# UZ-SLAMLab/DefSLAM

Measured on AMD Instinct MI355X. Metric: SfT GN iters/sec (500-node mesh, 1k matches), higher is better.
Workload: dtype f64

## Files before the change

defslam_amd/csrc/dsh_api.cpp:

```cpp
#include <hip/hip_runtime.h>

#include <algorithm>
#include <cmath>
#include <cstdio>
#include <cstdlib>
#include <cstring>

#include <memory>
#include <mutex>
#include <string>
#include <vector>

#include "dsh_sft_ctx.h"

#include "mapping_launch.h"

#ifdef DSH_LAB
#include "../../include/defslam_hip_debug.h"
#endif

LdsMarks g_lds_marks[64];
std::mutex g_lds_mu;

using dsh::Tcw_from_pose7;

dsh_ctx_base* dsh_base(dsh_ctx* ctx) { return static_cast<dsh_ctx_base*>(ctx); }
const dsh::TemplateHost* dsh_facet_template(dsh_ctx_base* c) {
  const dsh_ctx* x = static_cast<const dsh_ctx*>(c);
  return x && x->tmpl.valid && x->tmpl.F > 0 ? &x->tmpl : nullptr;
}

namespace {

void drop_graphs(dsh_ctx* c) {
  if (!c->host_only && c->stream) (void)hipStreamSynchronize(c->stream);
  for (auto& g : c->graphs)
    if (g->d_base) (void)hipFree(g->d_base);
  c->graphs.clear();
  c->packed.clear();
}

int upload_template(dsh_ctx* c) {
  c->B = 0;
  c->ran = false;
  drop_graphs(c);
  if (c->host_only) return DSH_OK;
  const dsh::TemplateHost& t = c->tmpl;
  Arena a;
  const size_t o_xyz0 = a.take(sizeof(double) * 3 * t.n);
  const size_t o_ptr = a.take(sizeof(int32_t) * (t.n + 1));
  const size_t o_idx = a.take(sizeof(int32_t) * t.nbr_idx.size());
  const size_t o_w = a.take(sizeof(double) * t.nbr_w.size());
  const size_t o_sw = a.take(sizeof(double) * t.n);
  const size_t o_k0 = a.take(sizeof(double) * t.n);
  if (c->d_tmpl) { (void)hipFree(c->d_tmpl); c->d_tmpl = nullptr; }
  HIPCHK(c, hipMalloc((void**)&c->d_tmpl, a.size));
  c->d_tmpl_bytes = a.size;
  std::vector<char> st(a.size, 0);
  std::memcpy(&st[o_xyz0], t.xyz0.data(), sizeof(double) * 3 * t.n);
  std::memcpy(&st[o_ptr], t.nbr_ptr.data(), sizeof(int32_t) * (t.n + 1));
  std::memcpy(&st[o_idx], t.nbr_idx.data(), sizeof(int32_t) * t.nbr_idx.size());
  std::memcpy(&st[o_w], t.nbr_w.data(), sizeof(double) * t.nbr_w.size());
  std::memcpy(&st[o_sw], t.nbr_sumw.data(), sizeof(double) * t.n);
  std::memcpy(&st[o_k0], t.k0.data(), sizeof(double) * t.n);
  HIPCHK(c, hipMemcpy(c->d_tmpl, st.data(), a.size, hipMemcpyHostToDevice));
  c->dt.xyz0 = (const double*)(c->d_tmpl + o_xyz0);
  c->dt.nbr_ptr = (const int32_t*)(c->d_tmpl + o_ptr);
  c->dt.nbr_idx = (const int32_t*)(c->d_tmpl + o_idx);
  c->dt.nbr_w = (const double*)(c->d_tmpl + o_w);
  c->dt.nbr_sumw = (const double*)(c->d_tmpl + o_sw);
  c->dt.k0 = (const double*)(c->d_tmpl + o_k0);
  return DSH_OK;
}

template <class T>
size_t reserve(Arena& a, const std::vector<T>& v) { return a.take(sizeof(T) * v.size()); }
template <class T>
void put(char* st, size_t off, const std::vector<T>& v) {
  if (!v.empty()) std::memcpy(st + off, v.data(), sizeof(T) * v.size());
}

int graph_for(dsh_ctx* c, const std::vector<uint8_t>& opt, dsh::SftGraph** out, std::string& err) {
  uint64_t h = 1469598103934665603ull;
  for (uint8_t b : opt) { h ^= b; h *= 1099511628211ull; }
  for (auto& g : c->graphs)
    if (g->opt_hash == h && g->opt == opt) { g->last_use = c->upload_serial; *out = g.get(); return DSH_OK; }
  if (c->graphs.size() >= 64) {
    if (!c->host_only && c->stream) (void)hipStreamSynchronize(c->stream);
    auto& gs = c->graphs;
    for (size_t i = 0; i < gs.size();) {
      if (gs[i]->last_use != c->upload_serial) {
        if (gs[i]->d_base) (void)hipFree(gs[i]->d_base);
        gs.erase(gs.begin() + i);
      } else {
        i++;
      }
    }
  }
  std::unique_ptr<dsh::SftGraph> g(new dsh::SftGraph());
  const int rc = dsh::build_graph(c->tmpl, opt, *g, err);
  if (rc != DSH_OK) return rc;
  g->last_use = c->upload_serial;
  if (!c->host_only) {
    Arena a;
    auto& o = g->o;
    o.act = reserve(a, g->act); o.actnode = reserve(a, g->actnode); o.star_node = reserve(a, g->star_node); o.star_sL = reserve(a, g->star_sL);
    o.str_nodes = reserve(a, g->str_nodes); o.str_L0 = reserve(a, g->str_L0); o.off_ptr = reserve(a, g->off_ptr); o.off_rc = reserve(a, g->off_rc);
    o.sh_ptr = reserve(a, g->sh_ptr); o.sh_rec = reserve(a, g->sh_rec); o.sh_cf = reserve(a, g->sh_cf); o.tmask = reserve(a, g->tmask);
    o.hgather = reserve(a, g->hgather);
    o.hgatherT = reserve(a, g->hgatherT);
    std::vector<char> st(a.size, 0);
    put(st.data(), o.act, g->act); put(st.data(), o.actnode, g->actnode); put(st.data(), o.star_node, g->star_node); put(st.data(), o.star_sL, g->star_sL);
    put(st.data(), o.str_nodes, g->str_nodes); put(st.data(), o.str_L0, g->str_L0); put(st.data(), o.off_ptr, g->off_ptr); put(st.data(), o.off_rc, g->off_rc);
    put(st.data(), o.sh_ptr, g->sh_ptr); put(st.data(), o.sh_rec, g->sh_rec); put(st.data(), o.sh_cf, g->sh_cf); put(st.data(), o.tmask, g->tmask);
    put(st.data(), o.hgather, g->hgather);
    put(st.data(), o.hgatherT, g->hgatherT);
    if (hipMalloc((void**)&g->d_base, a.size) != hipSuccess) { err = "out of device memory (graph)"; return DSH_ERR_HIP; }
    g->d_bytes = a.size;
    if (hipMemcpy(g->d_base, st.data(), a.size, hipMemcpyHostToDevice) != hipSuccess) { (void)hipFree(g->d_base); err = "graph upload failed"; return DSH_ERR_HIP; }
  }
  *out = g.get();
  c->graphs.push_back(std::move(g));
  return DSH_OK;
}

int pack_problem(dsh_ctx* c, const dsh_sft_frame& f, Packed& P, std::string& err) {
  const dsh::TemplateHost& t = c->tmpl;
  std::vector<uint8_t> viewed, opt;
  int rc = dsh::frame_active_set(t, f, viewed, opt, err);
  if (rc != DSH_OK) return rc;
  rc = graph_for(c, opt, &P.g, err);
  if (rc != DSH_OK) return rc;
  const dsh::SftGraph& g = *P.g;
  rc = dsh::pack_frame(t, g, f, viewed, P.f, err);
  if (rc != DSH_OK) return rc;
  SftDev& h = P.h;
  h = SftDev{};
  h.n = t.n; h.nA = g.nA; h.Dn = 3 * g.nA; h.kd = g.kd; h.ldh = h.kd + 1;
  h.M = f.M; h.V = P.f.V; h.S = g.S; h.Es = g.Es; h.noff = g.noff; h.max_iters = f.max_iters; h.mode = 0;
  h.fx = f.K[0]; h.fy = f.K[1]; h.cx = f.K[2]; h.cy = f.K[3];
  h.w_ref = f.reg_temp / std::pow(t.median_L, 2);
  h.w_curv = f.reg_lap / (double)g.nA;
  h.w_str = g.Es > 0 ? f.reg_inex / (double)g.Es : 0.0;
  const float deltaMono = (float)std::sqrt(5.991);
  h.hub_delta = (double)deltaMono;
  h.hub_dsqr = h.hub_delta * h.hub_delta;
  return DSH_OK;
}

int run_rounds_enqueue(dsh_ctx* c);
int run_rounds(dsh_ctx* c) {
  const int rc = run_rounds_enqueue(c);
  if (rc != DSH_OK)
    for (int s = 0; s < c->plan.n_sub; s++) if (c->sub_stream[s]) (void)hipStreamSynchronize(c->sub_stream[s]);
  return rc;
}
int run_rounds_enqueue(dsh_ctx* c) {
  const int B = c->B, S = c->plan.n_sub;
  int b0[kSftMaxSub + 1];
  for (int s = 0; s <= S; s++) b0[s] = (int)((long long)B * s / S);
  int tail_below = -1;
  if (S == 1 && c->opt.tail != 0) {
    if (c->opt.tail > 0) tail_below = c->opt.tail * c->num_cus;
    else tail_below = std::min(4 * c->num_cus, std::max(2 * c->num_cus, (int)((long long)3 * B / 4)));
  }
  auto launch = [&](int s, int phase) {
    const bool ev = c->phase_events && S == 1;
    if (ev) { hipEvent_t e; if (hipEventCreate(&e) == hipSuccess) { (void)hipEventRecord(e, c->stream); c->phase_events->push_back(e); c->phase_ids.push_back(phase); } }
    hipError_t r;
    {
      LDS_LOCK();
      if (phase == SFTB_PH_TAIL) r = sftb_tail_launch(c->d_probs + b0[s], c->d_runs + b0[s], c->d_counters + 16 * s, b0[s + 1] - b0[s], c->plan.max_kd, c->plan.jl_doubles, &LDS_MARKS(c).tail, c->num_cus, tail_below, c->sub_stream[s]);
      else r = sftb_launch(c->d_probs + b0[s], c->d_runs + b0[s], c->d_counters + 16 * s, c->d_linlist + b0[s], b0[s + 1] - b0[s], phase, c->plan.jl_doubles, c->plan.xyz_doubles, LDS_MARKS(c).b,
                           c->num_cus, tail_below, c->sub_stream[s]);
    }
    if (ev) { hipEvent_t e; if (hipEventCreate(&e) == hipSuccess) { (void)hipEventRecord(e, c->stream); c->phase_events->push_back(e); } }
    return r;
  };
  if (S > 1) {
    HIPCHK(c, hipEventRecord(c->sub_event[0], c->stream));
    for (int s = 1; s < S; s++) HIPCHK(c, hipStreamWaitEvent(c->sub_stream[s], c->sub_event[0], 0));
  }
  for (int s = 0; s < S; s++) HIPCHK(c, launch(s, SFTB_PH_INIT));
  const int worst = std::max(1, c->plan.max_iters_batch) * 10 + 1;
  int rounds = 0, group = std::max(1, std::min(worst, c->rounds_hint));
  if (tail_below >= B) group = 0;
  HIPCHK(c, c->spec_done.ensure(64 * kSftMaxSub, true));
  int rc = DSH_OK;
  while (true) {
    for (int i = 0; i < group && rounds < worst; i++, rounds++)
      for (int s = 0; s < S; s++) {
        HIPCHK(c, launch(s, SFTB_PH_LIN));
        HIPCHK(c, launch(s, SFTB_PH_FACTOR));
        HIPCHK(c, launch(s, SFTB_PH_TRIAL));
      }
    if (tail_below >= 0) HIPCHK(c, launch(0, SFTB_PH_TAIL));
    for (int s = 0; s < S; s++) HIPCHK(c, hipMemcpyAsync(c->spec_done.p + 64 * s, c->d_counters + 16 * s, 8 * sizeof(int), hipMemcpyDeviceToHost, c->sub_stream[s]));
    for (int s = 0; s < S; s++) HIPCHK(c, hipStreamSynchronize(c->sub_stream[s]));
    int done = 0;
    for (int s = 0; s < S; s++) done += *reinterpret_cast<const int*>(c->spec_done.p + 64 * s);
    const int* c0 = reinterpret_cast<const int*>(c->spec_done.p);
    if (done >= B) { c->rounds_hint = (tail_below >= 0 && c0[6]) ? std::max(1, c0[7]) : rounds; break; }
    if (rounds >= worst) { rc = dsh_fail(c, DSH_ERR_STATE, "batched rounds: a problem did not terminate within its trial budget"); break; }
    group = 2;
  }
  return rc;
}

int run_once(dsh_ctx* c) {
  if (c->plan.rounds_mode) return run_rounds(c);
  if (c->plan.K <= 1) {
    LDS_LOCK();
    HIPCHK(c, sft_lm_launch(c->d_probs, c->B, c->plan.max_kd, c->plan.jl_doubles, c->plan.nw, LDS_MARKS(c).lm, c->stream));
    return DSH_OK;
  }
  const int K = c->plan.K, B = c->B;
  HIPCHK(c, hipMemsetAsync(c->d_spec, 0, sizeof(SftSpec) * (size_t)B * K, c->stream));
  const int rounds_per_iter = (10 + K - 1) / K;
  const int worst = c->plan.max_iters_batch * rounds_per_iter;
  auto launch = [&](int phase) { LDS_LOCK(); return sft_spec_launch(c->d_probs, c->d_spec, B, K, phase, c->plan.nh, c->opt.owner_waves, c->plan.max_kd, c->plan.jl_doubles, LDS_MARKS(c).spec, c->stream); };
  if (c->plan.nh > 0) HIPCHK(c, hipMemsetAsync(c->d_sync, 0, c->layout.sync_total, c->stream));
  HIPCHK(c, launch(SFT_SPEC_INIT));
  int rounds = 0, group = std::max(2, std::min(worst, c->spec_hint));
  HIPCHK(c, c->spec_done.ensure(sizeof(SftSpec) * (size_t)B, true));
  while (true) {
    for (int i = 0; i < group && rounds < worst; i++, rounds++) {
      HIPCHK(c, launch(SFT_SPEC_LIN));
      if (c->plan.any_split) {
        HIPCHK(c, launch(SFT_SPEC_FACTOR));
        HIPCHK(c, launch(SFT_SPEC_SOLVE));
      }
      HIPCHK(c, launch(SFT_SPEC_TRIAL));
    }
    HIPCHK(c, launch(SFT_SPEC_LIN));
    HIPCHK(c, hipMemcpyAsync(c->spec_done.p, c->d_spec, sizeof(SftSpec) * (size_t)B, hipMemcpyDeviceToHost, c->stream));
    HIPCHK(c, hipStreamSynchronize(c->stream));
    const SftSpec* sp = reinterpret_cast<const SftSpec*>(c->spec_done.p);
    bool all_done = true;
    int needed = 0;
    for (int b = 0; b < B; b++) { all_done = all_done && sp[b].done; needed = std::max(needed, sp[b].launches); }
    if (all_done) { c->spec_hint = needed; break; }
    if (rounds >= worst) return dsh_fail(c, DSH_ERR_STATE, "speculative trials: a problem did not terminate within its launch budget");
    group = 2;
  }
  return DSH_OK;
}


SftBatchLayout layout_batch(const SftBatchPlan& plan, const std::vector<Packed>& packed, int B) {
  const int K = plan.K, nh = plan.nh;
  SftBatchLayout L;
  Arena a;
  L.o_tab = a.take(sizeof(SftDev) * B * K);
  L.ro.resize(B);
  for (int b = 0; b < B; b++) {
    const dsh::SftFramePack& F = packed[b].f;
    SftBatchLayout::ReadOnly& o = L.ro[b];
    o.obs_nodes = reserve(a, F.obs_nodes); o.obs_bary = reserve(a, F.obs_bary); o.obs_uv = reserve(a, F.obs_uv); o.obs_w = reserve(a, F.obs_w);
    o.ob_ptr = reserve(a, F.ob_ptr); o.ob_m = reserve(a, F.ob_m); o.ob_c = reserve(a, F.ob_c); o.viewed = reserve(a, F.viewed);
    o.xyz_init = reserve(a, F.xyz_init);
    o.pose_init = a.take(8 * 8);
  }
  L.ro_bytes = a.size;
  L.res_off = a.size;
  (void)a.take(sizeof(SftResHdr) * (size_t)B);
  L.res_offs.resize(B);
  for (int b = 0; b < B; b++) {
    const SftDev& h = packed[b].h;
    SftBatchLayout::Result& r = L.res_offs[b];
    r.xyz = a.take(8 * 3 * (size_t)h.n) - L.res_off; r.chi2 = a.take(8 * (size_t)h.M) - L.res_off;
    r.trace = a.take(8 * DSH_TRACE_STRIDE * DSH_MAX_ITERS) - L.res_off;
    r.mp = a.take(4 * 3 * (size_t)h.M) - L.res_off; r.outl = a.take((size_t)h.M) - L.res_off;
  }
  L.res_bytes = a.size - L.res_off;
  L.ws.resize((size_t)B * K);
  L.ws_off = a.size;
  L.o_spec = a.take(sizeof(SftSpec) * (size_t)B * K);
  L.o_runs = a.take(plan.rounds_mode ? sizeof(SftRun) * (size_t)B + 64 * kSftMaxSub + sizeof(int) * (size_t)B : 0);
  if (nh > 0)
    for (int e = 0; e < B * K; e++) {
      const SftProblemPlan& p = plan.prob[e % B];
      if (p.split) for (int g = 0; g < 2; g++) L.sync_total += Arena::round((size_t)4 * (16 + p.part[g].nT));
    }
  L.o_sync = a.take(L.sync_total);
  size_t sync_used = 0;
  for (int e = 0; e < B * K; e++) {
    const int b = e % B, lane = e / B;
    const SftDev& h = packed[b].h;
    const SftProblemPlan& p = plan.prob[b];
    const size_t Dnp = (size_t)((h.Dn + kNB - 1) / kNB) * kNB;
    SftBatchLayout::Work& w = L.ws[e];
    w.sx0 = a.take(K > 1 ? 8 * 3 * (size_t)h.n : 0); w.sx1 = a.take(K > 1 ? 8 * 3 * (size_t)h.n : 0);
    w.shadow_xyz = a.take(lane ? 8 * 3 * (size_t)h.n : 0); w.shadow_chi2 = a.take(lane ? 8 * (size_t)h.M : 0); w.shadow_hdr = a.take(lane ? sizeof(SftResHdr) : 0);
    w.bak = a.take(8 * 3 * (size_t)h.n);
    w.camrec = a.take(8 * (size_t)h.M * SFT_CAM_STRIDE);
    w.wtv = a.take(p.lds_class >= 1 ? 0 : 8 * ((size_t)h.M + 1)); w.Jstar = a.take(p.lds_class >= 1 ? 0 : 8 * 4 * (size_t)h.S);
    w.Anode = a.take(p.lds_class >= 2 ? 0 : 8 * 6 * (size_t)h.nA); w.Jstr = a.take(p.lds_class >= 2 ? 0 : 8 * 4 * (size_t)h.Es);
    const size_t band_elems = p.tile_mode ? (Dnp / kTS + SFT_H_PAD_TILE_ROWS) * (size_t)p.tpr * kTS * kTS : Dnp * (size_t)h.ldh;
    const size_t bord_elems = (SFT_BORDER + 1) * Dnp + SFT_H_PAD_BORDER;
    w.Hc = a.take(p.tile_mode == 1 ? 8 * packed[b].g->hc_elems() : 0);
    w.Hb = a.take(p.tile_mode == 1 ? 0 : 8 * band_elems); w.Hbord = a.take(8 * bord_elems); w.Hcn = a.take(8 * 56);
    w.Lb = a.take(8 * band_elems); w.Lbord = a.take(8 * bord_elems); w.Lc = a.take(8 * 56);
    w.Linv = a.take(8 * (Dnp / kTS) * (size_t)kTS * kTS);
    w.Lt = a.take(p.tile_mode == 2 ? 8 * band_elems : 0); w.LbT = a.take(p.tile_mode == 2 ? 8 * (Dnp / kTS) * (size_t)kTS * kTS : 0);
    w.x = a.take(8 * (Dnp + 8)); w.dbg = a.take(1024);
    if (p.split)
      for (int g = 0; g < 4; g++) {
        const SftPart& q = p.part[g];
        const size_t tiles = 8 * (size_t)q.nT * q.tpr * kTS * kTS, col = 8 * (size_t)q.nT * kTS * kTS;
        SftBatchLayout::Part& po = w.part[g];
        po.Hb = a.take(g < 2 && lane == 0 ? tiles : 0);
        po.Lb = a.take(tiles); po.Lt = a.take(tiles); po.LbT = a.take(col); po.Linv = a.take(col);
        po.Lbord = a.take(8 * 8 * (size_t)kTS * q.nT); po.x = a.take(8 * ((size_t)kTS * q.nT + 8)); po.xchg = a.take(8 * (size_t)p.sp_xl);
        const bool helped = nh > 0 && g < 2;
        po.Pf = a.take(helped ? tiles : 0); po.PfB = a.take(helped ? col : 0);
        po.sync = L.o_sync + sync_used;
        if (helped) sync_used += Arena::round((size_t)4 * (16 + q.nT));
      }
  }
  L.size = a.size;
  return L;
}

void stage_read_only(char* st, const SftBatchLayout& L, const std::vector<Packed>& packed, int B) {
  for (int b = 0; b < B; b++) {
    const dsh::SftFramePack& F = packed[b].f;
    const SftBatchLayout::ReadOnly& o = L.ro[b];
    put(st, o.obs_nodes, F.obs_nodes); put(st, o.obs_bary, F.obs_bary); put(st, o.obs_uv, F.obs_uv); put(st, o.obs_w, F.obs_w);
    put(st, o.ob_ptr, F.ob_ptr); put(st, o.ob_m, F.ob_m); put(st, o.ob_c, F.ob_c); put(st, o.viewed, F.viewed); put(st, o.xyz_init, F.xyz_init);
    std::memcpy(st + o.pose_init, F.pose_init, 7 * sizeof(double));
  }
}

SftDev bind_entry(const std::vector<Packed>& packed, const dsh_ctx::TemplateDev& dt, char* base, const SftBatchLayout& L, const SftBatchPlan& plan, int B, int e) {
  const int b = e % B, lane = e / B;
  const dsh::SftGraph& g = *packed[b].g;
  const SftBatchLayout::ReadOnly& o = L.ro[b];
  const SftBatchLayout::Result& r = L.res_offs[b];
  const SftBatchLayout::Work& w = L.ws[e];
  SftDev h = packed[b].h;
  plan.prob[b].apply(h);
  char* rbase = base + L.res_off;
  SftResHdr* d_hdr = (SftResHdr*)rbase;
  const char* gb = g.d_base;
  h.xyz0 = dt.xyz0; h.nbr_ptr = dt.nbr_ptr; h.nbr_idx = dt.nbr_idx; h.nbr_w = dt.nbr_w; h.nbr_sumw = dt.nbr_sumw; h.k0 = dt.k0;
  h.act = (const int32_t*)(gb + g.o.act); h.actnode = (const int32_t*)(gb + g.o.actnode); h.star_node = (const int32_t*)(gb + g.o.star_node);
  h.star_sL = (const double*)(gb + g.o.star_sL); h.str_nodes = (const int32_t*)(gb + g.o.str_nodes); h.str_L0 = (const double*)(gb + g.o.str_L0);
  h.off_ptr = (const int32_t*)(gb + g.o.off_ptr); h.off_rc = (const int32_t*)(gb + g.o.off_rc); h.sh_ptr = (const int32_t*)(gb + g.o.sh_ptr);
  h.sh_rec = (const uint32_t*)(gb + g.o.sh_rec); h.sh_cf = (const double*)(gb + g.o.sh_cf); h.tmask = (const int32_t*)(gb + g.o.tmask);
  h.hgather = (const uint32_t*)(gb + g.o.hgather);
  h.hgatherT = (const uint32_t*)(gb + g.o.hgatherT);
  h.obs_nodes = (const int32_t*)(base + o.obs_nodes); h.obs_bary = (const double*)(base + o.obs_bary);
  h.obs_uv = (const double*)(base + o.obs_uv); h.obs_w = (const double*)(base + o.obs_w);
  h.ob_ptr = (const int32_t*)(base + o.ob_ptr); h.ob_m = (const int32_t*)(base + o.ob_m); h.ob_c = (const double*)(base + o.ob_c);
  h.viewed = (const uint8_t*)(base + o.viewed);
  h.xyz_init = (const double*)(base + o.xyz_init); h.pose_init = (const double*)(base + o.pose_init);
  h.res = d_hdr + b; h.pose = d_hdr[b].pose;
  h.xyz = (double*)(rbase + r.xyz); h.chi2_obs = (double*)(rbase + r.chi2); h.trace = (double*)(rbase + r.trace);
  h.mappoint = (float*)(rbase + r.mp); h.outlier = (uint8_t*)(rbase + r.outl);
  h.xyz_bak = (double*)(base + w.bak);
  h.camrec = (double*)(base + w.camrec); h.wtv = (double*)(base + w.wtv); h.Anode = (double*)(base + w.Anode);
  h.Jstar = (double*)(base + w.Jstar); h.Jstr = (double*)(base + w.Jstr);
  h.Hc = (double*)(base + w.Hc); h.Hb = (double*)(base + w.Hb); h.Hbord = (double*)(base + w.Hbord); h.Hcorner = (double*)(base + w.Hcn);
  h.Lb = (double*)(base + w.Lb); h.Lbord = (double*)(base + w.Lbord); h.Lcorner = (double*)(base + w.Lc); h.Linv = (double*)(base + w.Linv);
  h.Lt = (double*)(base + w.Lt); h.LbT = (double*)(base + w.LbT);
  h.x = (double*)(base + w.x); h.dbg = (double*)(base + w.dbg);
  h.spec_xyz[0] = (double*)(base + w.sx0); h.spec_xyz[1] = (double*)(base + w.sx1);
  if (h.split)
    for (int g = 0; g < 4; g++) {
      const SftBatchLayout::Part& po = w.part[g];
      SftPart& q = h.part[g];
      q.Hb = g < 2 ? (double*)(base + L.ws[b].part[g].Hb) : (double*)(base + po.xchg);
      q.Lb = (double*)(base + po.Lb); q.Lt = (double*)(base + po.Lt); q.LbT = (double*)(base + po.LbT); q.Linv = (double*)(base + po.Linv);
      q.Lbord = (double*)(base + po.Lbord); q.x = (double*)(base + po.x); q.xchg = (double*)(base + po.xchg);
      const bool helped = plan.nh > 0 && g < 2;
      q.Pf = helped ? (double*)(base + po.Pf) : nullptr; q.PfB = helped ? (double*)(base + po.PfB) : nullptr;
      q.sync = helped ? (int32_t*)(base + po.sync) : nullptr;
    }
  if (lane) {
    h.xyz = (double*)(base + w.shadow_xyz); h.chi2_obs = (double*)(base + w.shadow_chi2);
    h.res = (SftResHdr*)(base + w.shadow_hdr); h.pose = ((SftResHdr*)(base + w.shadow_hdr))->pose;
    h.trace = nullptr; h.mappoint = nullptr; h.outlier = nullptr;
    if (h.tile_mode == 1 || h.split) {
      const SftBatchLayout::Work& w0 = L.ws[b];
      h.Hc = (double*)(base + w0.Hc); h.Hbord = (double*)(base + w0.Hbord); h.Hcorner = (double*)(base + w0.Hcn);
    }
  }
  return h;
}

int sub_streams(dsh_ctx* c, int want) {
  for (int i = 1; i < want; i++)
    if (!c->sub_stream[i] && hipStreamCreateWithFlags(&c->sub_stream[i], hipStreamNonBlocking) != hipSuccess) c->sub_stream[i] = nullptr;
  for (int i = 0; i < want; i++) if (!c->sub_stream[i] || !c->sub_event[0]) return 1;
  return want;
}

}

int dsh_sft_upload(dsh_ctx* c, int B, const dsh_sft_frame* frames, SftUploadMode mode) {
  if (!c || B <= 0 || !frames) return dsh_fail(c, DSH_ERR_ARG, "dsh_sft_batch_upload: bad argument");
  if (!c->tmpl.valid) return dsh_fail(c, DSH_ERR_STATE, "dsh_sft_batch_upload: no template");
  if (!c->host_only) (void)hipSetDevice(c->device);
  c->B = 0;
  c->ran = false;
  c->upload_serial++;
  if ((int)c->packed.size() != B) c->packed.resize(B);
  std::vector<SftSizes> sizes(B);
  for (int b = 0; b < B; b++) {
    std::string e;
    const int rc = pack_problem(c, frames[b], c->packed[b], e);
    if (rc != DSH_OK) return dsh_fail(c, rc, "problem " + std::to_string(b) + ": " + e);
    const SftDev& h = c->packed[b].h;
    sizes[b] = SftSizes{h.n, h.nA, h.Dn, h.kd, h.M, h.S, h.Es, h.max_iters};
  }
  SftBatchPlan plan = sft_plan_batch(sizes.data(), B, c->num_cus, c->opt, c->host_only, mode);
  if (c->host_only) {
    c->h_probs.resize(B);
    for (int b = 0; b < B; b++) { c->h_probs[b] = c->packed[b].h; plan.prob[b].apply(c->h_probs[b]); }
    c->plan = std::move(plan);
    c->B = B;
    return DSH_OK;
  }
  if (sft_lm_kernel_lds_bytes(plan.max_kd, plan.jl_doubles) > 160 * 1024 || plan.max_kd + kNB + SFT_BORDER > SFT_NT)
    return dsh_fail(c, DSH_ERR_ARG, "half-bandwidth too large for the LDS panel / workgroup");
  if (plan.n_sub > 1) plan.n_sub = sub_streams(c, plan.n_sub);
  SftBatchLayout L = layout_batch(plan, c->packed, B);
  bool fresh_arena = false;
  if (L.size > c->d_batch_cap) {
    HIPCHK(c, hipStreamSynchronize(c->stream));
    if (c->d_batch) { (void)hipFree(c->d_batch); c->d_batch = nullptr; c->d_batch_cap = 0; }
    HIPCHK(c, hipMalloc((void**)&c->d_batch, L.size));
    c->d_batch_cap = L.size;
    fresh_arena = true;
  }
  if (c->stage_busy) { HIPCHK(c, hipEventSynchronize(c->stage_free)); c->stage_busy = false; }
  HIPCHK(c, c->stage.ensure(L.ro_bytes, true));
  char* st = c->stage.p;
  char* base = c->d_batch;
  const size_t entries = (size_t)B * plan.K;
  c->h_probs.resize(entries);
  for (size_t e = 0; e < entries; e++) c->h_probs[e] = bind_entry(c->packed, c->dt, base, L, plan, B, (int)e);
  std::memcpy(st + L.o_tab, c->h_probs.data(), sizeof(SftDev) * entries);
  stage_read_only(st, L, c->packed, B);
  HIPCHK(c, hipMemcpyAsync(base, st, L.ro_bytes, hipMemcpyHostToDevice, c->stream));
  HIPCHK(c, hipEventRecord(c->stage_free, c->stream));
  c->stage_busy = true;
  if (fresh_arena) HIPCHK(c, hipMemsetAsync(base + L.ws_off, 0, L.size - L.ws_off, c->stream));
  HIPCHK(c, hipMemsetAsync(base + L.res_off, 0, L.res_bytes, c->stream));
  c->d_probs = (SftDev*)(base + L.o_tab);
  c->d_spec = (SftSpec*)(base + L.o_spec);
  c->d_runs = (SftRun*)(base + L.o_runs);
  c->d_counters = (int*)(base + L.o_runs + sizeof(SftRun) * (size_t)B);
  c->d_linlist = c->d_counters + 16 * kSftMaxSub;
  c->d_sync = base + L.o_sync;
  c->plan = std::move(plan);
  c->layout = std::move(L);
  c->B = B;
  return DSH_OK;
}

extern "C" {

int dsh_create(dsh_ctx** out, int device) {
  if (!out) return DSH_ERR_ARG;
  *out = nullptr;
  if (device == -1) {
    dsh_ctx* hc = new dsh_ctx();
    hc->device = -1;
    hc->host_only = true;
    *out = hc;
    return DSH_OK;
  }
  int count = 0;
  if (hipGetDeviceCount(&count) != hipSuccess || count <= 0) return DSH_ERR_NO_DEVICE;
  if (device < 0 || device >= count) return DSH_ERR_ARG;
  dsh_ctx* c = new dsh_ctx();
  c->device = device;
  if (hipSetDevice(device) != hipSuccess || hipStreamCreateWithFlags(&c->stream, hipStreamNonBlocking) != hipSuccess) {
    delete c;
    return DSH_ERR_HIP;
  }
  if (hipEventCreateWithFlags(&c->stage_free, hipEventDisableTiming) != hipSuccess) {
    (void)hipStreamDestroy(c->stream);
    delete c;
    return DSH_ERR_HIP;
  }
  int cus = 0;
  if (hipDeviceGetAttribute(&cus, hipDeviceAttributeMultiprocessorCount, device) == hipSuccess && cus > 0) c->num_cus = cus;
  c->sub_stream[0] = c->stream;
  if (hipEventCreateWithFlags(&c->sub_event[0], hipEventDisableTiming) != hipSuccess) c->sub_event[0] = nullptr;
  *out = c;
  return DSH_OK;
}

int dsh_destroy(dsh_ctx* c) {
  if (!c) return DSH_ERR_ARG;
  dsh_detach_stores(c);
  if (c->host_only) { c->stage.release(); c->results.release(); delete c; return DSH_OK; }
  (void)hipSetDevice(c->device);
  drop_graphs(c);
  for (int i = 1; i < kSftMaxSub; i++) if (c->sub_stream[i]) { (void)hipStreamSynchronize(c->sub_stream[i]); (void)hipStreamDestroy(c->sub_stream[i]); }
  for (int i = 0; i < kSftMaxSub; i++) if (c->sub_event[i]) (void)hipEventDestroy(c->sub_event[i]);
  if (c->stream) { (void)hipStreamSynchronize(c->stream); (void)hipStreamDestroy(c->stream); }
  if (c->stage_free) (void)hipEventDestroy(c->stage_free);
  c->stage.release();
  c->results.release();
  c->spec_done.release();
  if (c->d_tmpl) (void)hipFree(c->d_tmpl);
  c->scratch.release();
  c->pin_in.release();
  c->pin_out.release();
  if (c->d_batch) (void)hipFree(c->d_batch);
  if (c->d_sc) (void)hipFree(c->d_sc);
  delete c;
  return DSH_OK;
}

const char* dsh_last_error(const dsh_ctx* c) { return c ? c->err.c_str() : "null context"; }
void* dsh_stream(dsh_ctx* c) { return c ? (void*)c->stream : nullptr; }
int dsh_synchronize(dsh_ctx* c) {
  if (const int rc = dsh_enter(c, "dsh_synchronize")) return rc;
  HIPCHK(c, hipStreamSynchronize(c->stream));
  return DSH_OK;
}

int dsh_template_build(dsh_ctx* c, int n, const double* xyz0, int F, const int32_t* facets) {
  if (!c || n <= 0 || F <= 0 || !xyz0 || !facets) return dsh_fail(c, DSH_ERR_ARG, "dsh_template_build: bad argument");
  for (int i = 0; i < 3 * F; i++)
    if (facets[i] < 0 || facets[i] >= n) return dsh_fail(c, DSH_ERR_ARG, "dsh_template_build: facet index out of range");
  if (!c->host_only) (void)hipSetDevice(c->device);
  c->tmpl.build(n, xyz0, F, facets);
  return upload_template(c);
}

int dsh_template_set(dsh_ctx* c, int n, const double* xyz0, const uint8_t* boundary, const int32_t* rp, const int32_t* col, const double* w,
                     const double* k0, int E, const int32_t* en, const double* eL, double median_L) {
  if (!c || n <= 0 || E < 0 || !xyz0 || !boundary || !rp || !col || !w || !k0 || !en || !eL) return dsh_fail(c, DSH_ERR_ARG, "dsh_template_set: bad argument");
  if (rp[0] != 0) return dsh_fail(c, DSH_ERR_ARG, "dsh_template_set: nbr_rowptr[0] != 0");
  for (int i = 0; i < n; i++)
    if (rp[i + 1] < rp[i]) return dsh_fail(c, DSH_ERR_ARG, "dsh_template_set: nbr_rowptr is not non-decreasing");
  for (int p = 0; p < rp[n]; p++)
    if (col[p] < 0 || col[p] >= n) return dsh_fail(c, DSH_ERR_ARG, "dsh_template_set: neighbour index out of range");
  for (int e = 0; e < E; e++) {
    if (en[2 * e] < 0 || en[2 * e] >= n || en[2 * e + 1] < 0 || en[2 * e + 1] >= n) return dsh_fail(c, DSH_ERR_ARG, "dsh_template_set: edge node out of range");
    if (!(eL[e] > 0.0)) return dsh_fail(c, DSH_ERR_ARG, "dsh_template_set: edge rest length must be positive");
  }
  if (!(median_L > 0.0)) return dsh_fail(c, DSH_ERR_ARG, "dsh_template_set: median edge length must be positive");
  if (!c->host_only) (void)hipSetDevice(c->device);
  c->tmpl.set(n, xyz0, boundary, rp, col, w, k0, E, en, eL, median_L);
  return upload_template(c);
}

int dsh_template_dims(const dsh_ctx* c, int32_t* n, int32_t* E, int32_t* nnz) {
  if (!c || !c->tmpl.valid) return DSH_ERR_STATE;
  if (n) *n = c->tmpl.n;
  if (E) *E = c->tmpl.E;
  if (nnz) *nnz = (int32_t)c->tmpl.nbr_idx.size();
  return DSH_OK;
}

int dsh_template_get(const dsh_ctx* c, uint8_t* boundary, int32_t* rp, int32_t* col, double* w, double* k0, int32_t* en, double* eL, double* med) {
  if (!c || !c->tmpl.valid) return DSH_ERR_STATE;
  const dsh::TemplateHost& t = c->tmpl;
  if (boundary) std::memcpy(boundary, t.boundary.data(), t.n);
  if (rp) std::memcpy(rp, t.nbr_ptr.data(), sizeof(int32_t) * (t.n + 1));
  if (col) std::memcpy(col, t.nbr_idx.data(), sizeof(int32_t) * t.nbr_idx.size());
  if (w) std::memcpy(w, t.nbr_w.data(), sizeof(double) * t.nbr_w.size());
  if (k0) std::memcpy(k0, t.k0.data(), sizeof(double) * t.n);
  if (en) std::memcpy(en, t.edge_nodes.data(), sizeof(int32_t) * 2 * t.E);
  if (eL) std::memcpy(eL, t.edge_L0.data(), sizeof(double) * t.E);
  if (med) *med = t.median_L;
  return DSH_OK;
}

int dsh_template_embed(const dsh_ctx* c, int P, const float* pts, int32_t* facet_id, int32_t* nodes, float* bary) {
  if (!c || !c->tmpl.valid || c->tmpl.F <= 0) return DSH_ERR_STATE;
  if (P < 0 || !pts || !facet_id || !nodes || !bary) return DSH_ERR_ARG;
  c->tmpl.embed(P, pts, facet_id, nodes, bary);
  return DSH_OK;
}

int dsh_template_embed_device(dsh_ctx* c, int P, const float* pts, int32_t* facet_id, int32_t* nodes, float* bary) {
  if (!c) return DSH_ERR_ARG;
  if (!c->tmpl.valid || c->tmpl.F <= 0) return dsh_fail(c, DSH_ERR_STATE, "dsh_template_embed_device: needs a template built from facets");
  if (P < 0 || (P > 0 && (!pts || !facet_id || !nodes || !bary))) return dsh_fail(c, DSH_ERR_ARG, "dsh_template_embed_device: bad argument");
  if (c->host_only) return dsh_fail(c, DSH_ERR_NO_DEVICE, "dsh_template_embed_device: host-only context, no GPU (dsh_template_embed is the host routine)");
  if (P == 0) return DSH_OK;
  if (const int rc = dsh_enter(c, "dsh_template_embed_device")) return rc;
  const dsh::TemplateHost& t = c->tmpl;
  const size_t Pz = (size_t)P;
  UpBlock up;
  const size_t o_pts = up.copy_of(pts, 12 * Pz), o_xyz = up.copy_of(t.xyz0.data(), 24 * (size_t)t.n), o_fac = up.copy_of(t.facets.data(), 12 * (size_t)t.F),
               o_ptr = up.copy_of(t.nf_ptr.data(), 4 * (size_t)(t.n + 1)), o_idx = up.copy_of(t.nf_idx.data(), 4 * t.nf_idx.size());
  DownBlock down;
  const size_t d_fid = down.copy_to(facet_id, 4 * Pz), d_nodes = down.copy_to(nodes, 12 * Pz), d_bary = down.copy_to(bary, 12 * Pz);
  if (const int rc = up.copy(c)) return rc;
  if (const int rc = down.alloc(c)) return rc;
  HIPCHK(c, reg_embed(P, up.dev<float>(o_pts), t.n, up.dev<double>(o_xyz), up.dev<int32_t>(o_fac), up.dev<int32_t>(o_ptr), up.dev<int32_t>(o_idx),
                      down.dev<int32_t>(d_fid), down.dev<int32_t>(d_nodes), down.dev<float>(d_bary), c->stream));
  return down.receive(c);
}

int dsh_sft_batch_upload(dsh_ctx* c, int B, const dsh_sft_frame* frames) { return dsh_sft_upload(c, B, frames, SftUploadMode::batch); }

int dsh_sft_batch_run(dsh_ctx* c) {
  if (!c) return DSH_ERR_ARG;
  if (const int rc = dsh_enter(c, "dsh_sft_batch_run")) return rc;
  if (c->B <= 0) return dsh_fail(c, DSH_ERR_STATE, "dsh_sft_batch_run: nothing uploaded");
  const int rc = run_once(c);
  if (rc != DSH_OK) return rc;
  c->ran = true;
  return DSH_OK;
}

int dsh_sft_batch_counts(dsh_ctx* c, int64_t* iters, int64_t* trials) {
  if (!c || c->B <= 0 || !c->ran) return DSH_ERR_STATE;
  if (const int rc = dsh_enter(c, "dsh_sft_batch_counts")) return rc;
  const size_t bytes = sizeof(SftResHdr) * (size_t)c->B;
  HIPCHK(c, c->results.ensure(std::max(bytes, c->results.cap), true));
  HIPCHK(c, hipMemcpyAsync(c->results.p, c->d_batch + c->layout.res_off, bytes, hipMemcpyDeviceToHost, c->stream));
  HIPCHK(c, hipStreamSynchronize(c->stream));
  const SftResHdr* hd = reinterpret_cast<const SftResHdr*>(c->results.p);
  int64_t it = 0, tr = 0;
  for (int b = 0; b < c->B; b++) { it += hd[b].iters; tr += hd[b].trials; }
  if (iters) *iters = it;
  if (trials) *trials = tr;
  return DSH_OK;
}

int dsh_sft_batch_problem_info(dsh_ctx* c, int b, int64_t* bytes, int32_t* counts) {
  if (!c || b < 0 || b >= c->B) return DSH_ERR_ARG;
  const Packed& P = c->packed[b];
  const SftDev& h = P.h;
  const int64_t M = h.M, n = h.n, C = P.g->n_curv_ref, E = h.Es, V = h.V;
  const int64_t reads = 60 * M + 24 * n + 88 + 92 * C + 16 * E + 28 * V;
  const int64_t writes = 8 * (30 * M + 21 * C + 6 * E + 9 * V) + 8 * (2 * M + C + E + 3 * V) + 8 * M;
  if (bytes) *bytes = reads + writes;
  if (counts) { counts[0] = h.M; counts[1] = h.nA; counts[2] = P.g->n_curv_ref; counts[3] = h.Es; counts[4] = h.V; counts[5] = 6 + h.Dn; counts[6] = h.kd; counts[7] = c->plan.rounds_mode ? 1 : c->plan.nw; counts[8] = P.g->noff; }
  return DSH_OK;
}

int dsh_sft_batch_download(dsh_ctx* c, int B, dsh_sft_result* res) {
  if (!c || !res || B != c->B) return dsh_fail(c, DSH_ERR_ARG, "dsh_sft_batch_download: bad argument");
  if (const int rc = dsh_enter(c, "dsh_sft_batch_download")) return rc;
  if (!c->ran) return dsh_fail(c, DSH_ERR_STATE, "dsh_sft_batch_download: no run");
  HIPCHK(c, c->results.ensure(c->layout.res_bytes, true));
  HIPCHK(c, hipMemcpyAsync(c->results.p, c->d_batch + c->layout.res_off, c->layout.res_bytes, hipMemcpyDeviceToHost, c->stream));
  HIPCHK(c, hipStreamSynchronize(c->stream));
  const char* rb = c->results.p;
  const SftResHdr* hd = reinterpret_cast<const SftResHdr*>(rb);
  for (int b = 0; b < B; b++) {
    const SftDev& h = c->h_probs[b];
    const Packed& P = c->packed[b];
    const SftBatchLayout::Result& o = c->layout.res_offs[b];
    dsh_sft_result& r = res[b];
    r.rep_error = hd[b].rep_error;
    r.inliers = hd[b].inliers;
    r.iters = hd[b].iters;
    r.trials = hd[b].trials;
    r.status = hd[b].status;
    r.dim = 6 + h.Dn;
    r.half_bandwidth = h.kd;
    if (r.chi2_obs) std::memcpy(r.chi2_obs, rb + o.chi2, 8 * (size_t)h.M);
    if (r.outlier) std::memcpy(r.outlier, rb + o.outl, (size_t)h.M);
    if (r.xyz) std::memcpy(r.xyz, rb + o.xyz, 8 * 3 * (size_t)h.n);
    if (r.pose7) std::memcpy(r.pose7, hd[b].pose, 8 * 7);
    if (r.Tcw) Tcw_from_pose7(hd[b].pose, r.Tcw);
    if (r.mappoint_xyz) std::memcpy(r.mappoint_xyz, rb + o.mp, 4 * 3 * (size_t)h.M);
    if (r.trace) {
      const size_t rows = (size_t)std::max(P.f.max_iters, 0), done = std::min(rows, (size_t)std::max(hd[b].iters, 0));
      std::memcpy(r.trace, rb + o.trace, 8 * DSH_TRACE_STRIDE * done);
      std::memset(r.trace + DSH_TRACE_STRIDE * done, 0, 8 * DSH_TRACE_STRIDE * (rows - done));
    }
  }
  return DSH_OK;
}

int dsh_sft_solve(dsh_ctx* c, const dsh_sft_frame* frame, dsh_sft_result* result) {
  if (!c || !frame || !result) return dsh_fail(c, DSH_ERR_ARG, "dsh_sft_solve: bad argument");
  int rc = dsh_sft_batch_upload(c, 1, frame);
  if (rc != DSH_OK) return rc;
  rc = dsh_sft_batch_run(c);
  if (rc != DSH_OK) return rc;
  return dsh_sft_batch_download(c, 1, result);
}

#ifdef DSH_LAB
namespace {
struct EventPair {
  hipEvent_t e0 = nullptr, e1 = nullptr;
  hipError_t create() { hipError_t e = hipEventCreate(&e0); return e != hipSuccess ? e : hipEventCreate(&e1); }
  ~EventPair() { if (e0) (void)hipEventDestroy(e0); if (e1) (void)hipEventDestroy(e1); }
};
}

int dsh_lab_set_option(dsh_ctx* c, const char* name, int value) {
  if (!c || !name) return DSH_ERR_ARG;
  const std::string k(name);
  if (k == "waves") { if (value != 0 && value != 4 && value != 8) return dsh_fail(c, DSH_ERR_ARG, "dsh_lab_set_option: waves is 0 (automatic), 4 or 8"); c->opt.waves = value; }
  else if (k == "dataflow") c->opt.dataflow = value != 0;
  else if (k == "wide_off") c->opt.wide_off = value != 0;
  else if (k == "rounds") c->opt.rounds = value != 0;
  else if (k == "streams") { if (value < 0 || value > kSftMaxSub) return dsh_fail(c, DSH_ERR_ARG, "dsh_lab_set_option: streams is 0 (automatic) or 1..4 sub-batches"); c->opt.streams = value; }
  else if (k == "split") { if (value < 0 || value > 2) return dsh_fail(c, DSH_ERR_ARG, "dsh_lab_set_option: split is 0 (off), 1 (wide bands only) or 2 (every band long enough)"); c->opt.split = value; }
  else if (k == "helpers_wbt") { if (value < 1 || value > 16) return dsh_fail(c, DSH_ERR_ARG, "dsh_lab_set_option: helpers_wbt is 1..16 (tiles of half-bandwidth from which parts get helper workgroups)"); c->opt.helpers_wbt = value; }
  else if (k == "owner_waves") { if (value != 8 && value != 16) return dsh_fail(c, DSH_ERR_ARG, "dsh_lab_set_option: owner_waves is 8 or 16 (wavefronts of a FACTOR workgroup with helpers)"); c->opt.owner_waves = value; }
  else if (k == "helpers") { if (value < -1 || value > 3) return dsh_fail(c, DSH_ERR_ARG, "dsh_lab_set_option: helpers is -1 (automatic) or 0..3 workgroups per part"); c->opt.helpers = value; }
  else if (k == "tail") { if (value < -1 || value > 8) return dsh_fail(c, DSH_ERR_ARG, "dsh_lab_set_option: tail is -1 (automatic), 0 (rounds to the end) or the number of problems per CU from which downwards the last problems go to the tail kernel"); c->opt.tail = value; }
  else if (k == "speculate") { if (value < 0 || value > SFT_SPEC_MAXK) return dsh_fail(c, DSH_ERR_ARG, "dsh_lab_set_option: speculate is 0 (automatic) or 1..4 lanes"); c->opt.speculate = value; }
  else return dsh_fail(c, DSH_ERR_ARG, "dsh_lab_set_option: unknown option " + k);
  return DSH_OK;
}

int dsh_lab_sft_solver_info(dsh_ctx* c, int b, int32_t* out8) {
  if (!c || !out8 || b < 0 || b >= c->B) return dsh_fail(c, DSH_ERR_ARG, "dsh_lab_sft_solver_info: bad argument");
  const SftDev& h = c->h_probs[b];
  out8[0] = h.split; out8[1] = h.sp_c0; out8[2] = h.sp_s; out8[3] = h.sp_n1p; out8[4] = h.sp_pad; out8[5] = c->plan.K; out8[6] = h.tile_mode; out8[7] = c->plan.nw;
  return DSH_OK;
}

int dsh_lab_sft_run_timed(dsh_ctx* c, int launches, double* total_ms) {
  if (!c || launches <= 0 || !total_ms) return dsh_fail(c, DSH_ERR_ARG, "dsh_lab_sft_run_timed: bad argument");
  if (const int rc = dsh_enter(c, "dsh_lab_sft_run_timed")) return rc;
  if (c->B <= 0) return dsh_fail(c, DSH_ERR_STATE, "dsh_lab_sft_run_timed: nothing uploaded");
  EventPair ev;
  HIPCHK(c, ev.create());
  HIPCHK(c, hipEventRecord(ev.e0, c->stream));
  for (int i = 0; i < launches; i++) { const int rc = run_once(c); if (rc != DSH_OK) return rc; }
  HIPCHK(c, hipEventRecord(ev.e1, c->stream));
  HIPCHK(c, hipEventSynchronize(ev.e1));
  float ms = 0.f;
  HIPCHK(c, hipEventElapsedTime(&ms, ev.e0, ev.e1));
  *total_ms = (double)ms;
  c->ran = true;
  return DSH_OK;
}

int dsh_lab_sft_assemble_timed(dsh_ctx* c, int launches, double* total_ms) {
  if (!c || launches <= 0 || !total_ms) return dsh_fail(c, DSH_ERR_ARG, "dsh_lab_sft_assemble_timed: bad argument");
  if (const int rc = dsh_enter(c, "dsh_lab_sft_assemble_timed")) return rc;
  if (c->B <= 0 || !c->ran) return dsh_fail(c, DSH_ERR_STATE, "dsh_lab_sft_assemble_timed: needs an uploaded batch that has run once");
  EventPair ev;
  HIPCHK(c, ev.create());
  HIPCHK(c, hipEventRecord(ev.e0, c->stream));
  for (int i = 0; i < launches; i++) HIPCHK(c, sft_assembly_launch(c->d_probs, c->B, c->plan.max_kd, c->plan.jl_doubles, c->plan.rounds_mode ? 8 : c->plan.nw, c->stream));
  HIPCHK(c, hipEventRecord(ev.e1, c->stream));
  HIPCHK(c, hipEventSynchronize(ev.e1));
  float ms = 0.f;
  HIPCHK(c, hipEventElapsedTime(&ms, ev.e0, ev.e1));
  *total_ms = ms;
  c->ran = false;
  return DSH_OK;
}

int dsh_lab_sft_wave_check(dsh_ctx* c, double rel, int launches, int only, double* x_ref, double* x_new, int32_t* ok2, double* ms2) {
  if (!c || launches <= 0 || !ms2) return dsh_fail(c, DSH_ERR_ARG, "dsh_lab_sft_wave_check: bad argument");
  if (const int rc = dsh_enter(c, "dsh_lab_sft_wave_check")) return rc;
  if (c->B <= 0 || !c->ran) return dsh_fail(c, DSH_ERR_STATE, "dsh_lab_sft_wave_check: needs an uploaded batch that has run once");
  for (int b = 0; b < c->B; b++)
    if (c->h_probs[b].tile_mode != 1) return dsh_fail(c, DSH_ERR_STATE, "dsh_lab_sft_wave_check: register-window problems (half-bandwidth <= 128) only");
  HIPCHK(c, sft_assembly_launch(c->d_probs, c->B, c->plan.max_kd, c->plan.jl_doubles, c->plan.rounds_mode ? 8 : c->plan.nw, c->stream));
  EventPair ev;
  HIPCHK(c, ev.create());
  for (int which = 0; which < 2; which++) {
    if (only == 2 - which) continue;
    HIPCHK(c, sft_wave_lab_launch(c->d_probs, c->B, which, rel, c->plan.max_kd, c->plan.jl_doubles, c->stream));
    HIPCHK(c, hipEventRecord(ev.e0, c->stream));
    for (int i = 0; i < launches; i++) HIPCHK(c, sft_wave_lab_launch(c->d_probs, c->B, which, rel, c->plan.max_kd, c->plan.jl_doubles, c->stream));
    HIPCHK(c, hipEventRecord(ev.e1, c->stream));
    HIPCHK(c, hipEventSynchronize(ev.e1));
    float ms = 0.f;
    HIPCHK(c, hipEventElapsedTime(&ms, ev.e0, ev.e1));
    ms2[which] = (double)ms / launches;
    double* dst = which == 0 ? x_ref : x_new;
    size_t off = 0;
    for (int b = 0; b < c->B; b++) {
      const SftDev& h = c->h_probs[b];
      const size_t Dnp = (size_t)((h.Dn + kNB - 1) / kNB) * kNB;
      if (dst) HIPCHK(c, hipMemcpy(dst + off, h.x, 8 * (Dnp + 6), hipMemcpyDeviceToHost));
      off += Dnp + 6;
      double flag = 0.0;
      if (ok2) { HIPCHK(c, hipMemcpy(&flag, h.dbg + 2, 8, hipMemcpyDeviceToHost)); ok2[2 * b + which] = (int32_t)flag; }
    }
  }
  return DSH_OK;
}

int dsh_lab_sft_factor_check(dsh_ctx* c, const double* lambda, const uint8_t* factor, int grid, double* x, int32_t* ok) {
  if (!c || !lambda || grid < 0) return dsh_fail(c, DSH_ERR_ARG, "dsh_lab_sft_factor_check: bad argument");
  if (const int rc = dsh_enter(c, "dsh_lab_sft_factor_check")) return rc;
  if (c->B <= 0 || !c->ran) return dsh_fail(c, DSH_ERR_STATE, "dsh_lab_sft_factor_check: needs an uploaded batch that has run once");
  for (int b = 0; b < c->B; b++)
    if (c->h_probs[b].tile_mode != 1) return dsh_fail(c, DSH_ERR_STATE, "dsh_lab_sft_factor_check: register-window problems (half-bandwidth <= 128) only");
  const int B = c->B;
  struct OwnedDevBuf { void* p = nullptr; ~OwnedDevBuf() { if (p) (void)hipFree(p); } } runs, counters;
  HIPCHK(c, hipMalloc(&runs.p, sizeof(SftRun) * (size_t)B));
  HIPCHK(c, hipMalloc(&counters.p, 16 * sizeof(int)));
  std::vector<SftRun> h_runs(B);
  for (int b = 0; b < B; b++) {
    SftRun& R = h_runs[b];
    std::memset(&R, 0, sizeof(R));
    R.lambda = lambda[b];
    R.state = (!factor || factor[b]) ? SFTB_TRIAL : SFTB_DONE;
    R.fact_ok = -1;
  }
  HIPCHK(c, sft_assembly_launch(c->d_probs, B, c->plan.max_kd, c->plan.jl_doubles, c->plan.rounds_mode ? 8 : c->plan.nw, c->stream));
  for (int b = 0; b < B; b++) HIPCHK(c, hipMemcpyAsync(c->h_probs[b].dbg + 1, &lambda[b], sizeof(double), hipMemcpyHostToDevice, c->stream));
  HIPCHK(c, hipMemcpyAsync(runs.p, h_runs.data(), sizeof(SftRun) * (size_t)B, hipMemcpyHostToDevice, c->stream));
  HIPCHK(c, hipMemsetAsync(counters.p, 0, 16 * sizeof(int), c->stream));
  HIPCHK(c, sftb_factor_lab_launch(c->d_probs, (SftRun*)runs.p, (int*)counters.p, B, grid ? grid : std::min(B, 4 * c->num_cus), c->stream));
  HIPCHK(c, hipStreamSynchronize(c->stream));
  HIPCHK(c, hipMemcpy(h_runs.data(), runs.p, sizeof(SftRun) * (size_t)B, hipMemcpyDeviceToHost));
  size_t off = 0;
  for (int b = 0; b < B; b++) {
    const SftDev& h = c->h_probs[b];
    const size_t Dnp = (size_t)((h.Dn + kNB - 1) / kNB) * kNB;
    if (x) HIPCHK(c, hipMemcpy(x + off, h.x, 8 * (Dnp + 6), hipMemcpyDeviceToHost));
    off += Dnp + 6;
    if (ok) ok[b] = h_runs[b].fact_ok;
  }
  return DSH_OK;
}

int dsh_lab_sft_rounds_timed(dsh_ctx* c, double* ms4, int32_t* rounds) {
  if (!c || !ms4) return dsh_fail(c, DSH_ERR_ARG, "dsh_lab_sft_rounds_timed: bad argument");
  if (const int rc = dsh_enter(c, "dsh_lab_sft_rounds_timed")) return rc;
  if (c->B <= 0 || !c->plan.rounds_mode) return dsh_fail(c, DSH_ERR_STATE, "dsh_lab_sft_rounds_timed: needs an uploaded batch that runs as rounds of phase kernels");
  std::vector<hipEvent_t> ev;
  c->phase_events = &ev;
  c->phase_ids.clear();
  const int rc = run_rounds(c);
  c->phase_events = nullptr;
  (void)hipStreamSynchronize(c->stream);
  for (int i = 0; i < 7; i++) ms4[i] = 0.0;
  { int32_t cnt[16] = {0}; if (hipMemcpy(cnt, c->d_counters, sizeof(cnt), hipMemcpyDeviceToHost) == hipSuccess) { ms4[5] = (double)cnt[8]; ms4[6] = (double)cnt[9]; } }
  int n_trial = 0;
  for (size_t i = 0; i + 1 < ev.size(); i += 2) {
    float ms = 0.f;
    (void)hipEventElapsedTime(&ms, ev[i], ev[i + 1]);
    const int ph = c->phase_ids[i / 2];
    ms4[ph == SFTB_PH_INIT ? 0 : ph == SFTB_PH_LIN ? 1 : ph == SFTB_PH_FACTOR ? 2 : ph == SFTB_PH_TRIAL ? 3 : 4] += ms;
    n_trial += ph == SFTB_PH_TRIAL;
  }
  if (rounds) *rounds = n_trial;
  for (hipEvent_t e : ev) (void)hipEventDestroy(e);
  if (rc == DSH_OK) c->ran = true;
  return rc;
}

int dsh_lab_sft_dump(dsh_ctx* c, int b, int what, int64_t n, double* out) {
  if (!c || !out || b < 0 || b >= c->B || n <= 0) return dsh_fail(c, DSH_ERR_ARG, "dsh_lab_sft_dump: bad argument");
  if (const int rc = dsh_enter(c, "dsh_lab_sft_dump")) return rc;
  const SftDev& h = c->h_probs[b];
  const double* src = what == 0 ? h.Lb : what == 1 ? h.Linv : what == 2 ? h.Lbord : what == 3 ? h.Hc : what == 4 ? h.Hbord : what == 5 ? h.x : what == 6 ? h.Hcorner :
                      (what == 8 || what == 9) ? (const double*)h.part[what - 8].sync : h.dbg;
  if (!src) return dsh_fail(c, DSH_ERR_STATE, "dsh_lab_sft_dump: the problem has no such buffer");
  HIPCHK(c, hipStreamSynchronize(c->stream));
  HIPCHK(c, hipMemcpy(out, src, 8 * (size_t)n, hipMemcpyDeviceToHost));
  return DSH_OK;
}

int dsh_lab_sft_phase_ms(dsh_ctx* c, int b, double* out8) {
  if (!c || !out8 || b < 0 || b >= c->B) return dsh_fail(c, DSH_ERR_ARG, "dsh_lab_sft_phase_ms: bad argument");
  if (const int rc = dsh_enter(c, "dsh_lab_sft_phase_ms")) return rc;
  if (!c->ran) return dsh_fail(c, DSH_ERR_STATE, "dsh_lab_sft_phase_ms: no run");
#ifndef SFT_PHASE_TIMERS
  return dsh_fail(c, DSH_ERR_STATE, "dsh_lab_sft_phase_ms: this build has no phase timers (make lab EXTRA=-DSFT_PHASE_TIMERS)");
#else
  HIPCHK(c, hipStreamSynchronize(c->stream));
  HIPCHK(c, hipMemcpy(out8, c->h_probs[b].dbg, 8 * sizeof(double), hipMemcpyDeviceToHost));
  for (int i = 0; i < 8; i++) out8[i] *= 1e-5;
  {
    double as[6];
    HIPCHK(c, hipMemcpy(as, c->h_probs[b].dbg + 32, sizeof(as), hipMemcpyDeviceToHost));
    std::fprintf(stderr, "[lab] assembly sections of problem %d, kcycles of wave 0: corner %.0f, diagonal gather %.0f, butterfly+finish %.0f, off-diagonal %.0f, round overhead %.0f; rounds %.0f\n",
                 b, as[0] * 1e-3, as[1] * 1e-3, as[2] * 1e-3, as[3] * 1e-3, as[4] * 1e-3, as[5]);
  }
  return DSH_OK;
#endif
}

int dsh_lab_sft_step_trace(dsh_ctx* c, int b, double* out64) {
  if (!c || !out64 || b < 0 || b >= c->B) return dsh_fail(c, DSH_ERR_ARG, "dsh_lab_sft_step_trace: bad argument");
  if (const int rc = dsh_enter(c, "dsh_lab_sft_step_trace")) return rc;
  if (!c->ran) return dsh_fail(c, DSH_ERR_STATE, "dsh_lab_sft_step_trace: no run");
#ifndef SFT_STEP_TRACE
  return dsh_fail(c, DSH_ERR_STATE, "dsh_lab_sft_step_trace: this build has no step trace (make lab EXTRA=-DSFT_STEP_TRACE)");
#else
  HIPCHK(c, hipStreamSynchronize(c->stream));
  HIPCHK(c, hipMemcpy(out64, c->h_probs[b].dbg + 16, 64 * sizeof(double), hipMemcpyDeviceToHost));
  return DSH_OK;
#endif
}

int dsh_lab_sft_system(dsh_ctx* c, int b, int32_t D, double* H, double* bvec, double* chi2) {
  if (!c || b < 0 || b >= c->B) return dsh_fail(c, DSH_ERR_ARG, "dsh_lab_sft_system: bad argument");
  if (const int rc = dsh_enter(c, "dsh_lab_sft_system")) return rc;
  HIPCHK(c, hipStreamSynchronize(c->stream));
  SftDev h = c->h_probs[b];
  if (D != 6 + h.Dn) return dsh_fail(c, DSH_ERR_ARG, "dsh_lab_sft_system: D mismatch");
  const int32_t mode_saved = h.mode, split_saved = h.split;
  h.mode = 1;
  h.split = 0;
  HIPCHK(c, hipMemcpy(c->d_probs + b, &h, sizeof(SftDev), hipMemcpyHostToDevice));
  { LDS_LOCK(); HIPCHK(c, sft_lm_launch(c->d_probs + b, 1, c->plan.max_kd, c->plan.jl_doubles, c->plan.nw, LDS_MARKS(c).lm, c->stream)); }
  HIPCHK(c, hipStreamSynchronize(c->stream));
  c->ran = false;
  h.mode = mode_saved;
  h.split = split_saved;
  HIPCHK(c, hipMemcpy(c->d_probs + b, &h, sizeof(SftDev), hipMemcpyHostToDevice));
  const size_t Dnp = (size_t)((h.Dn + kNB - 1) / kNB) * kNB;
  const size_t band_elems = h.tile_mode ? (Dnp / kTS) * (size_t)h.tpr * kTS * kTS : Dnp * (size_t)h.ldh;
  std::vector<double> Hb(h.tile_mode == 1 ? 0 : band_elems), Hbord(SFT_BORDER * Dnp), Hc(56);
  auto hidx = [&](int r, int cc) -> size_t {
    const size_t tb = ((size_t)(r >> 4) * h.tpr + ((r >> 4) - (cc >> 4))) * (kTS * kTS);
    if (h.tile_mode == 1) return tb + ((((r & 15) & 3) << 4) + (cc & 15)) * 4 + ((r & 15) >> 2);
    if (h.tile_mode == 2) return tb + ((((cc & 15) & 3) << 4) + (r & 15)) * 4 + ((cc & 15) >> 2);
    return (size_t)r * h.ldh + (cc - r + h.kd);
  };
  const dsh::SftGraph& g = *c->packed[b].g;
  std::vector<double> Hcomp;
  if (h.tile_mode == 1) {
    Hcomp.resize(g.hc_elems());
    HIPCHK(c, hipMemcpy(Hcomp.data(), h.Hc, 8 * Hcomp.size(), hipMemcpyDeviceToHost));
  } else {
    HIPCHK(c, hipMemcpy(Hb.data(), h.Hb, 8 * Hb.size(), hipMemcpyDeviceToHost));
  }
  auto hval = [&](int r, int cc) -> double {
    if (h.tile_mode != 1) return Hb[hidx(r, cc)];
    const int I = r >> 4, d = I - (cc >> 4);
    if (d > kBT) return 0.0;
    const int lane = (((r & 15) & 3) << 4) + (cc & 15), q = (r & 15) >> 2;
    return Hcomp[g.hgather[(((size_t)I * (kBT + 1) + d) * 64 + lane) * 4 + q] / 8];
  };
  HIPCHK(c, hipMemcpy(Hbord.data(), h.Hbord, 8 * Hbord.size(), hipMemcpyDeviceToHost));
  HIPCHK(c, hipMemcpy(Hc.data(), h.Hcorner, 8 * 49, hipMemcpyDeviceToHost));
  if (chi2) HIPCHK(c, hipMemcpy(chi2, h.dbg, 8, hipMemcpyDeviceToHost));
  if (H) {
    std::fill(H, H + (size_t)D * D, 0.0);
    for (int r = 0; r < h.Dn; r++)
      for (int k = 0; k <= h.kd; k++) {
        const int cidx = r - h.kd + k;
        if (cidx < 0) continue;
        const double v = hval(r, cidx);
        H[(size_t)(6 + r) + (size_t)(6 + cidx) * D] = v;
        H[(size_t)(6 + cidx) + (size_t)(6 + r) * D] = v;
      }
    for (int k = 0; k < 6; k++)
      for (int r = 0; r < h.Dn; r++) {
        const double v = Hbord[(size_t)k * Dnp + r];
        H[(size_t)k + (size_t)(6 + r) * D] = v;
        H[(size_t)(6 + r) + (size_t)k * D] = v;
      }
    for (int r = 0; r < 6; r++)
      for (int k = 0; k <= r; k++) {
        H[(size_t)r + (size_t)k * D] = Hc[r * 7 + k];
        H[(size_t)k + (size_t)r * D] = Hc[r * 7 + k];
      }
  }
  if (bvec) {
    for (int r = 0; r < 6; r++) bvec[r] = Hc[42 + r];
    for (int r = 0; r < h.Dn; r++) bvec[6 + r] = Hbord[(size_t)6 * Dnp + r];
  }
  return DSH_OK;
}
#endif

}
```

defslam_amd/csrc/dsh_sft_ctx.h:

```cpp
#pragma once
#include <hip/hip_runtime.h>

#include <memory>
#include <mutex>
#include <string>
#include <vector>

#include "../../include/defslam_hip.h"
#include "dsh_ctx.h"
#include "dsh_template.h"
#include "sft_pack.h"
#include "sft_plan.h"
#include "sft_problem.h"

struct LdsMarks { size_t lm[2] = {0, 0}, sc = 0, spec[2] = {0, 0}, cn = 0, b[2] = {0, 0}, tail = 0; };
extern LdsMarks g_lds_marks[64];
extern std::mutex g_lds_mu;
#define LDS_MARKS(c) (g_lds_marks[(c)->device & 63])
#define LDS_LOCK() std::lock_guard<std::mutex> lds_lock__(g_lds_mu)

struct Packed {
  SftDev h{};
  dsh::SftGraph* g = nullptr;
  dsh::SftFramePack f;
};

struct dsh_ctx : dsh_ctx_base {
  dsh::TemplateHost tmpl;
  char* d_tmpl = nullptr;
  size_t d_tmpl_bytes = 0;
  struct TemplateDev {
    const double *xyz0, *nbr_w, *nbr_sumw, *k0;
    const int32_t *nbr_ptr, *nbr_idx;
  } dt{};
  std::vector<std::unique_ptr<dsh::SftGraph>> graphs;
  uint64_t upload_serial = 0;
  int B = 0;
  std::vector<Packed> packed;
  SftBatchPlan plan;
  SftBatchLayout layout;
  char* d_batch = nullptr;
  size_t d_batch_cap = 0;
  SftDev* d_probs = nullptr;
  std::vector<SftDev> h_probs;
  HostBuf stage;
  hipEvent_t stage_free = nullptr;
  bool stage_busy = false;
  HostBuf results;
  char* d_sync = nullptr;
  int spec_hint = 12;
  SftSpec* d_spec = nullptr;
  HostBuf spec_done;
  SftSc* d_sc = nullptr;
  SftRun* d_runs = nullptr;
  int* d_counters = nullptr;
  int* d_linlist = nullptr;
  int rounds_hint = 24;
  hipStream_t sub_stream[kSftMaxSub] = {nullptr, nullptr, nullptr, nullptr};
  hipEvent_t sub_event[kSftMaxSub] = {nullptr, nullptr, nullptr, nullptr};
  std::vector<hipEvent_t>* phase_events = nullptr;
  std::vector<int> phase_ids;
  int num_cus = 256;
  bool ran = false;
  SftOptions opt;
};

int dsh_sft_upload(dsh_ctx* c, int B, const dsh_sft_frame* frames, SftUploadMode mode);
```

defslam_amd/csrc/sft_batch.h:

```cpp
#pragma once

#define SFTB_NW 8
#ifndef SFTB_LIN_NW
#define SFTB_LIN_NW 8
#endif
#ifndef SFTB_LIN_WAVES
#define SFTB_LIN_WAVES 2
#endif
#ifndef SFTB_TRIAL_WAVES
#define SFTB_TRIAL_WAVES 2
#endif

__device__ __forceinline__ void sftb_ctl_lds(char* smem, Ctl*& ctl, double*& red, double*& out, double*& panel) {
  ctl = reinterpret_cast<Ctl*>(smem);
  red = reinterpret_cast<double*>(smem + 512);
  out = red + 16 * 27 + 5;
  panel = out + 32;
}

__global__ __launch_bounds__(64 * SFTB_NW, 2) void sftb_init_kernel(const SftDev* __restrict__ probs, SftRun* __restrict__ runs, int* __restrict__ counters, int* __restrict__ lin_list, int tail_below) {
  const SftDev& P = probs[blockIdx.x];
  if (blockIdx.x == 0 && threadIdx.x == 0 && (int)gridDim.x <= tail_below) counters[6] = 1;
  init_state<64 * SFTB_NW>(P);
  if (threadIdx.x == 0) {
    SftRun& R = runs[blockIdx.x];
    R.lambda = -1.0; R.ni = 2.0; R.chi_cur = 0.0; R.chi_ini = 0.0; R.rho = 0.0; R.lambda_start = 0.0;
    R.it = 0; R.qmax = 0; R.nbad = 0; R.accepted = 0; R.all_ok = 1; R.iters = 0; R.trials = 0; R.fact_ok = 1;
    R.state = P.max_iters > 0 ? SFTB_LIN : SFTB_FINISH;
    if (P.max_iters > 0) lin_list[atomicAdd(&counters[2], 1)] = blockIdx.x;
  }
}

template <int NW>
__device__ __forceinline__ void sftb_lin_problem(const SftDev& P, SftRun& R, Ctl* ctl, double* red, double* out, double* panel) {
  constexpr int NT = 64 * NW;
  const int tid = threadIdx.x;
  auto nothing = [] {};
  const double chi0 = linearise<NW, decltype(nothing), true>(P, ctl, red, out, panel, nothing);
  double lambda = R.lambda;
  if (R.it == 0) {
    double mx = 0.0;
    for (int r = tid; r < P.Dn; r += NT) mx = fmax(mx, fabs(h_diag(P, r)));
    if (tid < 6) mx = fmax(mx, fabs(P.Hcorner[tid * 8]));
    mx = block_max(mx, red);
    lambda = 1e-5 * mx;
  }
  if (tid == 0) {
    if (R.it == 0) { R.lambda = lambda; R.ni = 2.0; R.nbad = 0; }
    R.chi_cur = chi0; R.chi_ini = chi0; R.qmax = 0; R.rho = 0.0; R.accepted = 0; R.all_ok = 1; R.lambda_start = lambda;
    R.state = SFTB_TRIAL;
  }
}

__global__ __launch_bounds__(64 * SFTB_LIN_NW, SFTB_LIN_WAVES) void sftb_lin_kernel(const SftDev* __restrict__ probs, SftRun* __restrict__ runs, int* __restrict__ counters,
                                                                                  const int* __restrict__ lin_list, int B, int tail_below) {
  constexpr int NW = SFTB_LIN_NW, NT = 64 * NW;
  extern __shared__ __attribute__((aligned(16))) char smem[];
  __shared__ int next_b;
  Ctl* ctl; double *red, *out, *panel;
  sftb_ctl_lds(smem, ctl, red, out, panel);
  const int tid = threadIdx.x;
  if (counters[6] || B - counters[0] <= tail_below) {
    if (blockIdx.x == 0 && tid == 0) counters[6] = 1;
    return;
  }
  if (blockIdx.x == 0 && tid == 0) counters[7]++;
  auto fetch = [&]() { const int i = atomicAdd(&counters[3], 1); return i < counters[2] ? lin_list[i] : -1; };
  int nxt = -1;
  if (tid == 0) nxt = fetch();
  while (true) {
    if (tid == 0) next_b = nxt;
    __syncthreads();
    const int b = __builtin_amdgcn_readfirstlane(next_b);
    if (b < 0) break;
    if (tid == 0) { nxt = fetch(); atomicAdd(&counters[9], 1); }
    sftb_lin_problem<NW>(probs[b], runs[b], ctl, red, out, panel);
  }
}

__global__ __launch_bounds__(64, 1) void sftb_factor_kernel(const SftDev* __restrict__ probs, SftRun* __restrict__ runs, int* __restrict__ counters, int B) {
  extern __shared__ __attribute__((aligned(16))) char smem[];
  lds_double* lds = to_lds(reinterpret_cast<double*>(smem));
  const int lane = threadIdx.x;
  if (counters[6]) return;
  for (int i = lane; i < WV_LDS_DOUBLES; i += 64) lds[i] = 0.0;
  if (blockIdx.x == 0 && lane == 0) { counters[2] = 0; counters[3] = 0; }
  WvPrev Q;
  Q.Lg = nullptr; Q.Linv = nullptr; Q.x = nullptr; Q.nT = 0; Q.active = 0; Q.m8[0] = Q.m8[1] = 0; Q.xb = 0.0;
  int n_done = 0;
  while (true) {
    int b = 0;
    if (lane == 0) b = atomicAdd(&counters[1], 1);
    b = __builtin_amdgcn_readfirstlane(b);
    if (b >= B) break;
    if (runs[b].state != SFTB_TRIAL) continue;
    const SftDev& P = probs[b];
    const double lambda = runs[b].lambda;
    double xcam;
    const int ok = wv_factor(P, lambda, lambda, lds, Q, xcam);
    if (lane == 0) runs[b].fact_ok = ok;
    Q = wv_prev_of(P, ok, xcam, lane);
    n_done++;
  }
  int lane_now;
  asm volatile("v_mbcnt_lo_u32_b32 %0, -1, 0\n\tv_mbcnt_hi_u32_b32 %0, -1, %0" : "=v"(lane_now));
  if (Q.active) wv_backsub_now(Q, lane_now);
  if (lane_now == 0 && n_done) atomicAdd(&counters[8], n_done);
}

template <int NW>
__device__ __forceinline__ int sftb_trial_problem(const SftDev& P, SftRun& R, Ctl* ctl, double* red, double* out, double* panel, int* counters, int* lin_list, int b) {
  constexpr int NT = 64 * NW;
  const int tid = threadIdx.x;
  const int Dn = P.Dn;
  const int Dnp = ((Dn + NB - 1) / NB) * NB;
  const int ok = R.fact_ok;
  const double lam = R.lambda;
  const bool in_lds = P.lds_class >= 1;
  if (!in_lds)
    for (int i = tid; i < 3 * P.n; i += NT) {
      const double v = P.xyz[i];
      P.xyz_bak[i] = v;
      const int a = P.act[i / 3];
      if (a >= 0) P.xyz[i] = v + P.x[3 * a + (i % 3)];
    }
  if (tid < 7) R.pose_bak[tid] = P.pose[tid];
  __syncthreads();
  if (tid == 0) pose_oplus(P.pose, P.x + Dnp);
  double sc = 0.0;
  for (int r = tid; r < Dn; r += NT) { const double xv = P.x[r]; sc += xv * (lam * xv + P.Hbord[(size_t)6 * Dnp + r]); }
  if (tid < 6) { const double xv = P.x[Dnp + tid]; sc += xv * (lam * xv + P.Hcorner[42 + tid]); }
  __syncthreads();
  block_sum<1>(&sc, red, out);
  const double scale = out[0];
  __syncthreads();
  const auto staged = asm_records<NW, 1>(P, panel);
  const double chi_new = in_lds ? eval_edges<false, 1>(P, ctl, red, out, staged, P.x)
                                : eval_edges<false, 0>(P, ctl, red, out, asm_records<NW, 0>(P, panel));
  if (tid == 0) {
    const double tempChi = ok ? chi_new : DBL_MAX;
    double rho = (R.chi_cur - tempChi);
    rho /= (scale + 1e-3);
    R.rho = rho;
    if (rho > 0 && isfinite(tempChi)) {
      double alpha = 1. - pow((2 * rho - 1), 3);
      alpha = fmin(alpha, 2. / 3.);
      const double sf = fmax(1. / 3., alpha);
      R.lambda = lam * sf; R.ni = 2.0; R.chi_cur = tempChi; R.accepted = 1;
      ctl->stop = 0;
    } else {
      R.lambda = lam * R.ni; R.ni *= 2.0;
      ctl->stop = 1;
    }
    R.qmax++;
    R.all_ok &= ok;
    ctl->qmax = R.qmax;
    ctl->rho = rho;
  }
  __syncthreads();
  if (ctl->stop) {
    if (!in_lds)
      for (int i = tid; i < 3 * P.n; i += NT) P.xyz[i] = P.xyz_bak[i];
    if (tid < 7) P.pose[tid] = R.pose_bak[tid];
  } else if (in_lds) {
    for (int i = tid; i < 3 * P.n; i += NT) P.xyz[i] = staged.xyz_l[i];
  }
  const bool again = (ctl->rho < 0) && (ctl->qmax < 10);
  if (again) return 0;
  __syncthreads();
  if (tid == 0) {
    const int qmax = R.qmax;
    R.trials += qmax;
    R.iters++;
    if (P.trace) {
      double* t = P.trace + R.it * 8;
      t[0] = R.chi_ini; t[1] = R.lambda_start; t[2] = qmax; t[3] = R.chi_cur; t[4] = R.lambda; t[5] = R.rho; t[6] = R.accepted; t[7] = R.all_ok;
    }
    if (!R.all_ok) P.res->status |= 1;
    bool term = (qmax == 10) || (R.rho == 0);
    if (!term) {
      if ((R.chi_ini - R.chi_cur) * 1e3 < R.chi_ini) R.nbad++; else R.nbad = 0;
      term = R.nbad >= 3;
    }
    R.it++;
    if (R.it >= P.max_iters) term = true;
    ctl->nbad = term ? 1 : 0;
    ctl->it = R.iters;
    ctl->accepted = R.trials;
    R.state = term ? SFTB_DONE : SFTB_LIN;
    if (!term && lin_list) lin_list[atomicAdd(&counters[2], 1)] = b;
  }
  __syncthreads();
  if (ctl->nbad) {
    const int iters = ctl->it, trials = ctl->accepted;
    __syncthreads();
    classify<NT>(P, ctl, panel, iters, trials);
    if (tid == 0) atomicAdd(&counters[0], 1);
    return 2;
  }
  return 1;
}

__global__ __launch_bounds__(64 * SFTB_NW, SFTB_TRIAL_WAVES) void sftb_trial_kernel(const SftDev* __restrict__ probs, SftRun* __restrict__ runs, int* __restrict__ counters, int* __restrict__ lin_list) {
  constexpr int NW = SFTB_NW, NT = 64 * NW;
  SftRun& R = runs[blockIdx.x];
  const int st = R.state;
  if (counters[6]) return;
  if (blockIdx.x == 0 && threadIdx.x == 0) counters[1] = 0;
  if (st != SFTB_TRIAL && st != SFTB_FINISH) return;
  extern __shared__ __attribute__((aligned(16))) char smem[];
  const SftDev& P = probs[blockIdx.x];
  Ctl* ctl; double *red, *out, *panel;
  sftb_ctl_lds(smem, ctl, red, out, panel);
  const int tid = threadIdx.x;
  if (st == SFTB_FINISH) {
    classify<NT>(P, ctl, panel, 0, 0);
    if (tid == 0) { R.state = SFTB_DONE; atomicAdd(&counters[0], 1); }
    return;
  }
  (void)sftb_trial_problem<NW>(P, R, ctl, red, out, panel, counters, lin_list, blockIdx.x);
}

__device__ __noinline__ void sftb_solve8(const SftDev& P, unsigned ctl_off, unsigned ws_off, double lambda) {
  typedef __attribute__((address_space(3))) char lds_char;
  Ctl* ctl = reinterpret_cast<Ctl*>((char*)(lds_char*)(size_t)__builtin_amdgcn_readfirstlane(ctl_off));
  double* ws = reinterpret_cast<double*>((char*)(lds_char*)(size_t)__builtin_amdgcn_readfirstlane(ws_off));
  factor_tiles_df8<1>(P, ctl, ws, lambda, true);
  backsub_tiles<8>(P, ctl, ws);
}

__global__ __launch_bounds__(64 * SFTB_NW, SFT_WAVES_PER_EU) void sftb_tail_kernel(const SftDev* __restrict__ probs, SftRun* __restrict__ runs, int* __restrict__ counters, int B, int tail_below) {
  constexpr int NW = SFTB_NW, NT = 64 * NW;
  extern __shared__ __attribute__((aligned(16))) char smem[];
  Ctl* ctl; double *red, *out, *panel;
  sftb_ctl_lds(smem, ctl, red, out, panel);
  const int tid = threadIdx.x;
  if (!counters[6]) {
    if (B - counters[0] > tail_below) return;
    if (blockIdx.x == 0 && tid == 0) counters[6] = 1;
  }
  while (true) {
    __syncthreads();
    if (tid == 0) ctl->it = atomicAdd(&counters[5], 1);
    __syncthreads();
    const int b = __builtin_amdgcn_readfirstlane(ctl->it);
    __syncthreads();
    if (b >= B) break;
    SftRun& R = runs[b];
    const SftDev& P = probs[b];
    int st = R.state;
    if (st == SFTB_FINISH) {
      classify<NT>(P, ctl, panel, 0, 0);
      if (tid == 0) { R.state = SFTB_DONE; atomicAdd(&counters[0], 1); }
      continue;
    }
    while (st == SFTB_LIN || st == SFTB_TRIAL) {
      if (st == SFTB_LIN) {
        sftb_lin_problem<NW>(P, R, ctl, red, out, panel);
        __syncthreads();
      }
      if (tid == 0) ctl->lambda = R.lambda;
      __syncthreads();
      sftb_solve8(P, (unsigned)(size_t)(__attribute__((address_space(3))) char*)(char*)ctl, (unsigned)(size_t)(__attribute__((address_space(3))) char*)(char*)panel, R.lambda);
      if (tid == 0) R.fact_ok = ctl->fact_ok;
      __syncthreads();
      const int r = sftb_trial_problem<NW>(P, R, ctl, red, out, panel, counters, nullptr, b);
      __syncthreads();
      st = r == 0 ? SFTB_TRIAL : (r == 1 ? SFTB_LIN : SFTB_DONE);
    }
  }
}
```

defslam_amd/csrc/sft_kernels.hip:

```cpp
#include <hip/hip_runtime.h>
#include <type_traits>
#include <utility>
#include <algorithm>
#include <cstdio>
#include <cstdlib>
#include <math.h>
#include <float.h>
#define SFT_KERNEL_SOURCE
#include "sft_problem.h"
#include "tile_chol.h"

#define NB 32

#if defined(SFT_PHASE_TIMERS) && defined(DSH_LAB)
#define PH_T0() long long ph_t0__ = wall_clock64()
#define PH_ADD(slot)                                                          \
  do {                                                                        \
    const long long t1__ = wall_clock64();                                    \
    if (threadIdx.x == 0) P.dbg[slot] += (double)(t1__ - ph_t0__);            \
    ph_t0__ = t1__;                                                           \
  } while (0)
#define PH_RESET() ph_t0__ = wall_clock64()
#define AS_T0() long long as_t0__ = clock64()
#define AS_ADD(slot) do { const long long t1__ = clock64(); if (threadIdx.x == 0) P.dbg[slot] += (double)(t1__ - as_t0__); as_t0__ = t1__; } while (0)
// ... 2649 lines not shown
    if (tid == 0) {
      for (int i = 0; i < SFT_SC_XCHG; i++) S.send[i] = 0.0;
      S.send[0] = chi_new; S.send[1] = scale_nodes;
    }
  } else {
    if (tid == 0) {
      const int ok = S.fact_ok;
      S.all_ok &= ok;
      double scale = S.recv[1];
      for (int k = 0; k < 6; k++) { const double xv = P.x[Dnp + k]; scale += xv * (S.lambda * xv + S.bc[k]); }
      double tempChi = ok ? S.recv[0] : DBL_MAX;
      double rho = (S.chi_cur - tempChi);
      rho /= (scale + 1e-3);
      S.rho = rho;
      if (rho > 0 && isfinite(tempChi)) {
        double alpha = 1. - pow((2 * rho - 1), 3);
        alpha = fmin(alpha, 2. / 3.);
        const double sf = fmax(1. / 3., alpha);
        S.lambda *= sf; S.ni = 2.0; S.chi_cur = tempChi; S.accepted = 1;
        ctl->stop = 0;
      } else {
        S.lambda *= S.ni; S.ni *= 2.0;
        ctl->stop = 1;
      }
      S.qmax++;
    }
    __syncthreads();
    if (ctl->stop) {
      for (int i = tid; i < 3 * P.n; i += NT) P.xyz[i] = P.xyz_bak[i];
      if (tid < 7) P.pose[tid] = S.pose_bak[tid];
    }
    __syncthreads();
    const bool again = (S.rho < 0) && (S.qmax < 10);
    bool finished = false;
    if (!again) {
      if (tid == 0) {
        S.trials += S.qmax;
        S.iters++;
        if (P.trace) {
          double* t = P.trace + S.it * 8;
          t[0] = S.chi_ini; t[1] = S.lambda_start; t[2] = S.qmax; t[3] = S.chi_cur; t[4] = S.lambda; t[5] = S.rho; t[6] = S.accepted; t[7] = S.all_ok;
        }
        if (!S.all_ok) P.res->status |= 1;
        bool term = (S.qmax == 10) || (S.rho == 0);
        if (!term) {
          if ((S.chi_ini - S.chi_cur) * 1e3 < S.chi_ini) S.nbad++; else S.nbad = 0;
          term = S.nbad >= 3;
        }
        S.it++;
        if (S.it >= P.max_iters) term = true;
        S.done = term ? 1 : 0;
        ctl->qmax = term ? 1 : 0;
      }
      __syncthreads();
      finished = ctl->qmax != 0;
    }
    if (tid == 0) S.again = again ? 1 : 0;
    if (finished) classify<NT>(P, ctl, panel, S.iters, S.trials);
  }
}

template <int NW>
__global__ __launch_bounds__(64 * NW, SFT_WAVES_PER_EU) void sft_cn_kernel(const SftDev* __restrict__ probs, SftSc* __restrict__ scs, int phase) {
  constexpr int NT = 64 * NW;
  extern __shared__ __attribute__((aligned(16))) char smem[];
  const SftDev& P = probs[blockIdx.x];
  SftSc& S = scs[blockIdx.x];
  Ctl* ctl = reinterpret_cast<Ctl*>(smem);
  double* red = reinterpret_cast<double*>(smem + 512);
  double* out = red + 16 * 27 + 5;
  double* panel = out + 32;
  const int tid = threadIdx.x;
  const int Dn = P.Dn;
  const int Dnp = ((Dn + NB - 1) / NB) * NB;
  const int part = S.rank;
  if (phase == SFT_CN_LIN) {
    if (S.it == 0) {
      init_state<NT>(P);
      if (tid == 0) { S.lambda = -1.0; S.ni = 2.0; S.nbad = 0; S.iters = 0; S.trials = 0; S.done = 0; }
      __syncthreads();
    }
    const double chi0 = linearise<NW>(P, ctl, red, out, panel, [] {});
    if (S.it == 0) {
      double mx = 0.0;
      for (int r = tid; r < Dn; r += NT) mx = fmax(mx, fabs(h_diag(P, r)));
      if (tid < 6) mx = fmax(mx, fabs(P.Hcorner[tid * 8]));
      mx = block_max(mx, red);
      if (tid == 0) { S.lambda = 1e-5 * mx; S.ni = 2.0; S.nbad = 0; }
    }
    __syncthreads();
    if (tid == 0) { S.chi_cur = chi0; S.chi_ini = chi0; S.qmax = 0; S.rho = 0.0; S.accepted = 0; S.all_ok = 1; S.lambda_start = S.lambda; }
  } else if (phase == SFT_CN_FAC) {
    for (int i = tid; i < 3 * P.n; i += NT) P.xyz_bak[i] = P.xyz[i];
    if (tid < 7) S.pose_bak[tid] = P.pose[tid];
    if (tid == 0) ctl->lambda = S.lambda;
    __syncthreads();
    if constexpr (NW == 8) factor_wide(P, part, ctl, panel);
  } else if (phase == SFT_CN_SOL) {
    const int nTr = P.part[2].nT;
    const bool parts_ok = P.part[2].xchg[(size_t)nTr * P.part[2].tpr * (TS * TS) + (size_t)8 * TS * nTr + 56] == 0.0;
    if (tid == 0) ctl->lambda = S.lambda;
    __syncthreads();
    if constexpr (NW == 8) {
      if (parts_ok) factor_wide(P, 2, ctl, panel);
      else if (tid == 0) ctl->fact_ok = 0;
      __syncthreads();
      backsub_wide(P, 2, ctl, panel);
      backsub_wide(P, part, ctl, panel);
    }
    for (int i = tid; i < Dnp + 6; i += NT) P.x[i] = 0.0;
    __syncthreads();
    if (ctl->fact_ok) {
      const int c0 = P.sp_c0, sp = P.sp_s, pad = P.sp_pad, n1p = P.sp_n1p;
      const auto xa = P.part[part].x, xr = P.part[2].x;
      if (part == 0) {
        for (int j = tid; j < c0; j += NT) P.x[j] = xa[j];
        for (int k = tid; k < sp; k += NT) P.x[c0 + k] = xr[k];
        if (tid < 6) P.x[Dnp + tid] = xr[TS * nTr + tid];
      } else {
        for (int j = pad + tid; j < n1p; j += NT) P.x[Dn - 1 - (j - pad)] = xa[j];
      }
    }
    if (tid == 0) S.fact_ok = ctl->fact_ok;
  } else {
    for (int i = tid; i < 3 * P.n; i += NT) {
      const int a = P.act[i / 3];
      if (a >= 0) P.xyz[i] += P.x[3 * a + (i % 3)];
    }
    if (tid == 0) pose_oplus(P.pose, P.x + Dnp);
    double sc = 0.0;
    const double lam = S.lambda;
    for (int r = tid; r < Dn; r += NT) { const double xv = P.x[r]; sc += xv * (lam * xv + P.Hbord[(size_t)6 * Dnp + r]); }
    if (tid < 6) { const double xv = P.x[Dnp + tid]; sc += xv * (lam * xv + P.Hcorner[42 + tid]); }
    __syncthreads();
    block_sum<1>(&sc, red, out);
    const double scale = out[0];
    __syncthreads();
    const double chi_new = eval_edges<false, 0>(P, ctl, red, out, asm_records<NW, 0>(P, panel));
    if (tid == 0) {
      const int ok = S.fact_ok;
      S.all_ok &= ok;
      const double tempChi = ok ? chi_new : DBL_MAX;
      double rho = (S.chi_cur - tempChi);
      rho /= (scale + 1e-3);
      S.rho = rho;
      if (rho > 0 && isfinite(tempChi)) {
        double alpha = 1. - pow((2 * rho - 1), 3);
        alpha = fmin(alpha, 2. / 3.);
        const double sf = fmax(1. / 3., alpha);
        S.lambda *= sf; S.ni = 2.0; S.chi_cur = tempChi; S.accepted = 1;
        ctl->stop = 0;
      } else {
        S.lambda *= S.ni; S.ni *= 2.0;
        ctl->stop = 1;
      }
      S.qmax++;
    }
    __syncthreads();
    if (ctl->stop) {
      for (int i = tid; i < 3 * P.n; i += NT) P.xyz[i] = P.xyz_bak[i];
      if (tid < 7) P.pose[tid] = S.pose_bak[tid];
    }
    __syncthreads();
    const bool again = (S.rho < 0) && (S.qmax < 10);
    bool finished = false;
    if (!again) {
      if (tid == 0) {
        S.trials += S.qmax;
        S.iters++;
        if (P.trace) {
          double* t = P.trace + S.it * 8;
          t[0] = S.chi_ini; t[1] = S.lambda_start; t[2] = S.qmax; t[3] = S.chi_cur; t[4] = S.lambda; t[5] = S.rho; t[6] = S.accepted; t[7] = S.all_ok;
        }
        if (!S.all_ok) P.res->status |= 1;
        bool term = (S.qmax == 10) || (S.rho == 0);
        if (!term) {
          if ((S.chi_ini - S.chi_cur) * 1e3 < S.chi_ini) S.nbad++; else S.nbad = 0;
          term = S.nbad >= 3;
        }
        S.it++;
        if (S.it >= P.max_iters) term = true;
        S.done = term ? 1 : 0;
        ctl->qmax = term ? 1 : 0;
      }
      __syncthreads();
      finished = ctl->qmax != 0;
    }
    if (tid == 0) S.again = again ? 1 : 0;
    if (finished) classify<NT>(P, ctl, panel, S.iters, S.trials);
  }
}

#include "sft_batch.h"

#ifdef DSH_LAB
template <int NW>
__global__ __launch_bounds__(64 * NW, SFT_WAVES_PER_EU) void sft_assembly_kernel(const SftDev* __restrict__ probs) {
  constexpr int NT = 64 * NW;
  extern __shared__ __attribute__((aligned(16))) char smem[];
  const SftDev& P = probs[blockIdx.x];
  Ctl* ctl = reinterpret_cast<Ctl*>(smem);
  double* red = reinterpret_cast<double*>(smem + 512);
  double* out = red + 16 * 27 + 5;
  double* panel = out + 32;
  const int tid = threadIdx.x;
  for (int i = tid; i < 3 * P.n; i += NT) P.xyz[i] = P.xyz_init[i];
  if (tid < 7) P.pose[tid] = P.pose_init[tid];
  __syncthreads();
  double chi = 0.0;
  switch (P.lds_class) {
    case 3: { const auto jp = asm_records<NW, 3>(P, panel); chi = eval_edges<true, 3>(P, ctl, red, out, jp); assemble<NW, 3>(P, red, out, jp); break; }
    case 2: { const auto jp = asm_records<NW, 2>(P, panel); chi = eval_edges<true, 2>(P, ctl, red, out, jp); assemble<NW, 2>(P, red, out, jp); break; }
    case 1: { const auto jp = asm_records<NW, 1>(P, panel); chi = eval_edges<true, 1>(P, ctl, red, out, jp); assemble<NW, 1>(P, red, out, jp); break; }
    default: { const auto jp = asm_records<NW, 0>(P, panel); chi = eval_edges<true, 0>(P, ctl, red, out, jp); assemble<NW, 0>(P, red, out, jp); break; }
  }
  if (tid == 0) P.dbg[0] = chi;
}

template <int NW>
__device__ __forceinline__ void ref_factor_solve(const SftDev& P, Ctl* ctl, double* panel) {
  tile_factor<NW>(P, ctl, panel);
  backsub_tiles<NW>(P, ctl, panel);
}
template <int NW>
__global__ __launch_bounds__(64 * NW, SFT_WAVES_PER_EU) void sft_ref_solve_kernel(const SftDev* __restrict__ probs, double rel) {
  constexpr int NT = 64 * NW;
  extern __shared__ __attribute__((aligned(16))) char smem[];
  const SftDev& P = probs[blockIdx.x];
  Ctl* ctl = reinterpret_cast<Ctl*>(smem);
  double* red = reinterpret_cast<double*>(smem + 512);
  double* out = red + 16 * 27 + 5;
  double* panel = out + 32;
  const int tid = threadIdx.x;
  double mx = 0.0;
  for (int r = tid; r < P.Dn; r += NT) mx = fmax(mx, fabs(h_diag(P, r)));
  if (tid < 6) mx = fmax(mx, fabs(P.Hcorner[tid * 8]));
  mx = block_max(mx, red);
  if (tid == 0) { ctl->lambda = rel * 1e-5 * mx; P.dbg[1] = ctl->lambda; }
  __syncthreads();
  ref_factor_solve<NW>(P, ctl, panel);
  if (tid == 0) P.dbg[2] = ctl->fact_ok;
}
__global__ __launch_bounds__(64, 1) void sft_wave_solve_kernel(const SftDev* __restrict__ probs) {
  extern __shared__ __attribute__((aligned(16))) char smem[];
  const SftDev& P = probs[blockIdx.x];
  const double lambda = P.dbg[1];
  const int ok = wv_factor_solve(P, lambda, lambda, to_lds(reinterpret_cast<double*>(smem)));
  int lane_now;
  asm volatile("v_mbcnt_lo_u32_b32 %0, -1, 0\n\tv_mbcnt_hi_u32_b32 %0, -1, %0" : "=v"(lane_now));
  if (lane_now == 0) P.dbg[2] = ok;
}
#endif

}


extern "C" size_t sft_lm_kernel_lds_bytes(int kd, size_t jl_doubles) {
  const size_t rows = NB + kd + SFT_BORDER;
  const size_t LDP = rows | 1;
  size_t panel = (size_t)NB * LDP + 2 * NB * NB;
  const size_t backsub = NB + (SFT_NT / NB) * NB + NB * NB;
  if (backsub > panel) panel = backsub;
  const size_t tiles = (size_t)(BT + 2 * (BT + 1) + 3) * TILE_LDS + 3 * SFT_BORDER * TS + 64 + 48 + 128 + 128;
  if (kd <= TS * BT) panel = tiles;
  else if (kd <= TS * WB) panel = std::max(panel, std::max((size_t)2 * WB * TS * TS + TILE_LDS + 704, (size_t)(SFT_WIDE_NEAR + 2) * SFT_WIDE_NEAR * TS * TS + 2 * TILE_LDS + 704 + (size_t)32 * TS * TS + (size_t)(WB - SFT_WIDE_NEAR + 1) * TS * TS));
  if (jl_doubles > panel) panel = jl_doubles;
  return 512 + (16 * 27 + 5 + 32 + panel) * sizeof(double) + 64;
}

#ifdef DSH_LAB
extern "C" hipError_t sft_assembly_launch(const SftDev* d_probs, int B, int max_kd, size_t jl_doubles, int nw, hipStream_t stream) {
  const size_t lds = sft_lm_kernel_lds_bytes(max_kd, jl_doubles);
  const void* fn = nw == 4 ? reinterpret_cast<const void*>(sft_assembly_kernel<4>) : reinterpret_cast<const void*>(sft_assembly_kernel<8>);
  hipError_t e = hipFuncSetAttribute(fn, hipFuncAttributeMaxDynamicSharedMemorySize, (int)lds);
  if (e != hipSuccess) return e;
  if (nw == 4) hipLaunchKernelGGL(sft_assembly_kernel<4>, dim3(B), dim3(256), lds, stream, d_probs);
  else hipLaunchKernelGGL(sft_assembly_kernel<8>, dim3(B), dim3(512), lds, stream, d_probs);
  return hipGetLastError();
}
#endif

extern "C" hipError_t sft_sc_launch(const SftDev* d_probs, SftSc* d_sc, int B, int phase, int max_kd, size_t jl_doubles, size_t* configured, hipStream_t stream) {
  const size_t lds = sft_lm_kernel_lds_bytes(max_kd, jl_doubles);
  if (lds > *configured) {
    hipError_t e = hipFuncSetAttribute(reinterpret_cast<const void*>(sft_sc_kernel<8>), hipFuncAttributeMaxDynamicSharedMemorySize, (int)lds);
    if (e != hipSuccess) return e;
    *configured = lds;
  }
  hipLaunchKernelGGL(sft_sc_kernel<8>, dim3(B), dim3(512), lds, stream, d_probs, d_sc, phase);
  return hipGetLastError();
}

extern "C" hipError_t sft_cn_launch(const SftDev* d_probs, SftSc* d_sc, int phase, int max_kd, size_t jl_doubles, size_t* configured, hipStream_t stream) {
  const size_t lds = sft_lm_kernel_lds_bytes(max_kd, jl_doubles);
  if (lds > *configured) {
    hipError_t e = hipFuncSetAttribute(reinterpret_cast<const void*>(sft_cn_kernel<8>), hipFuncAttributeMaxDynamicSharedMemorySize, (int)lds);
    if (e != hipSuccess) return e;
    *configured = lds;
  }
  hipLaunchKernelGGL(sft_cn_kernel<8>, dim3(1), dim3(512), lds, stream, d_probs, d_sc, phase);
  return hipGetLastError();
}

extern "C" hipError_t sftb_tail_launch(const SftDev* d_probs, SftRun* d_runs, int* d_counters, int B, int max_kd, size_t jl_doubles, size_t* configured, int num_cus, int tail_below, hipStream_t stream) {
  const size_t lds = sft_lm_kernel_lds_bytes(max_kd, jl_doubles);
  if (lds > *configured) {
    hipError_t e = hipFuncSetAttribute(reinterpret_cast<const void*>(sftb_tail_kernel), hipFuncAttributeMaxDynamicSharedMemorySize, (int)lds);
    if (e != hipSuccess) return e;
    *configured = lds;
  }
  hipLaunchKernelGGL(sftb_tail_kernel, dim3(std::min(B, num_cus)), dim3(64 * SFTB_NW), lds, stream, d_probs, d_runs, d_counters, B, tail_below);
  return hipGetLastError();
}

#ifdef DSH_LAB
__global__ __launch_bounds__(1024) void sft_part_factor_kernel(const SftDev* __restrict__ probs, SftSpec* __restrict__ specs, int K, int nh) {
  constexpr int NT = 1024;
  extern __shared__ __attribute__((aligned(16))) char smem[];
  const int roles = 1 + nh, per_role = gridDim.x / roles;
  const int role = blockIdx.x / per_role, bid = blockIdx.x % per_role;
  const int fpart = bid % 2, bx = bid / 2;
  const int B = per_role / (K * 2), b = bx / K, j = bx % K;
  const SftDev& P = probs[(size_t)j * B + b];
  const SftSpec& S = specs[(size_t)j * B + b];
  Ctl* ctl = reinterpret_cast<Ctl*>(smem);
  double* red = reinterpret_cast<double*>(smem + 512);
  double* panel = red + 16 * 27 + 5 + 32;
  const int tid = threadIdx.x;
  if (S.done) return;
  if (!(P.tile_mode == 2 && P.split) || S.need_lin == 1) return;
  if (S.qbase + j >= 10) return;
  const int epoch = S.launches + 1;
  if (role > 0) {
    factor_wide_helper<16>(P, fpart, role - 1, nh, epoch, ctl, panel);
    return;
  }
  double lam = S.lambda, ni = S.ni;
  if (S.need_lin == 2 && S.it == 0) {
    double mx = 0.0;
    for (int r = tid; r < P.Dn; r += NT) mx = fmax(mx, fabs(h_diag(P, r)));
    if (tid < 6) mx = fmax(mx, fabs(P.Hcorner[tid * 8]));
    mx = block_max(mx, red);
    lam = 1e-5 * mx; ni = 2.0;
  }
  for (int t = 0; t < j; t++) { lam *= ni; ni *= 2.0; }
  if (tid == 0) ctl->lambda = lam;
  __syncthreads();
  factor_part<SFT_WIDE_NEAR, 16>(P, fpart, ctl, panel, epoch, nh);
}
#endif

__global__ void sft_vec_sum2_kernel(const double* a, const double* b, double* out_a, double* out_b, int n) {
  for (int i = blockIdx.x * blockDim.x + threadIdx.x; i < n; i += gridDim.x * blockDim.x) {
    const double v = a[i] + b[i];
    out_a[i] = v;
    out_b[i] = v;
  }
}
extern "C" hipError_t sft_vec_sum2(const double* a, const double* b, double* out_a, double* out_b, int n, hipStream_t stream) {
  hipLaunchKernelGGL(sft_vec_sum2_kernel, dim3(64), dim3(256), 0, stream, a, b, out_a, out_b, n);
  return hipGetLastError();
}

extern "C" hipError_t sft_spec_launch(const SftDev* d_probs, SftSpec* d_spec, int B, int K, int phase, int nh, int owner_waves, int max_kd, size_t jl_doubles, size_t* configured, hipStream_t stream) {
  const size_t lds = sft_lm_kernel_lds_bytes(max_kd, jl_doubles);
#ifdef DSH_LAB
  if (phase == SFT_SPEC_FACTOR && nh > 0 && owner_waves == 16) {
    if (lds > configured[1]) {
      hipError_t e = hipFuncSetAttribute(reinterpret_cast<const void*>(sft_part_factor_kernel), hipFuncAttributeMaxDynamicSharedMemorySize, (int)lds);
      if (e != hipSuccess) return e;
      configured[1] = lds;
    }
    hipLaunchKernelGGL(sft_part_factor_kernel, dim3(B * K * 2 * (1 + nh)), dim3(1024), lds, stream, d_probs, d_spec, K, nh);
    return hipGetLastError();
  }
#endif
  if (lds > *configured) {
    hipError_t e = hipFuncSetAttribute(reinterpret_cast<const void*>(sft_spec_kernel<8>), hipFuncAttributeMaxDynamicSharedMemorySize, (int)lds);
    if (e != hipSuccess) return e;
    *configured = lds;
  }
  const int wgs = (phase == SFT_SPEC_FACTOR || phase == SFT_SPEC_SOLVE) ? 2 : 1, roles = phase == SFT_SPEC_FACTOR ? 1 + nh : 1;
  hipLaunchKernelGGL(sft_spec_kernel<8>, dim3(B * K * wgs * roles), dim3(512), lds, stream, d_probs, d_spec, K, phase, nh);
  return hipGetLastError();
}

__global__ void sft_sc_local_reduce_kernel(SftSc* const* scs, int G) {
  const int i = threadIdx.x;
  if (i >= SFT_SC_XCHG) return;
  double s = 0.0;
  for (int g = 0; g < G; g++) s += scs[g]->send[i];
  for (int g = 0; g < G; g++) scs[g]->recv[i] = s;
}
extern "C" hipError_t sft_sc_local_reduce(SftSc* const* d_ptrs, int G, hipStream_t stream) {
  hipLaunchKernelGGL(sft_sc_local_reduce_kernel, dim3(1), dim3(64), 0, stream, d_ptrs, G);
  return hipGetLastError();
}

extern "C" hipError_t sft_lm_launch(const SftDev* d_probs, int B, int max_kd, size_t jl_doubles, int nw, size_t* configured, hipStream_t stream) {
  const size_t lds = sft_lm_kernel_lds_bytes(max_kd, jl_doubles);
  const int slot = nw == 4 ? 0 : 1;
  if (lds > configured[slot]) {
    const void* fn = nw == 4 ? reinterpret_cast<const void*>(sft_lm_kernel<4>) : reinterpret_cast<const void*>(sft_lm_kernel<8>);
    hipError_t e = hipFuncSetAttribute(fn, hipFuncAttributeMaxDynamicSharedMemorySize, (int)lds);
    if (e != hipSuccess) return e;
    configured[slot] = lds;
  }
  if (nw == 4) hipLaunchKernelGGL(sft_lm_kernel<4>, dim3(B), dim3(256), lds, stream, d_probs);
  else hipLaunchKernelGGL(sft_lm_kernel<8>, dim3(B), dim3(512), lds, stream, d_probs);
  return hipGetLastError();
}

#ifdef DSH_LAB
extern "C" hipError_t sft_wave_lab_launch(const SftDev* d_probs, int B, int which, double rel, int max_kd, size_t jl_doubles, hipStream_t stream) {
  if (which == 0) {
    (void)jl_doubles;
    const size_t lds = sft_lm_kernel_lds_bytes(max_kd, 0);
    hipError_t e = hipFuncSetAttribute(reinterpret_cast<const void*>(sft_ref_solve_kernel<4>), hipFuncAttributeMaxDynamicSharedMemorySize, (int)lds);
    if (e != hipSuccess) return e;
    hipLaunchKernelGGL(sft_ref_solve_kernel<4>, dim3(B), dim3(256), lds, stream, d_probs, rel);
  } else {
    hipLaunchKernelGGL(sft_wave_solve_kernel, dim3(B), dim3(64), WV_LDS_DOUBLES * sizeof(double), stream, d_probs);
  }
  return hipGetLastError();
}
#endif

extern "C" hipError_t sftb_launch(const SftDev* d_probs, SftRun* d_runs, int* d_counters, int* d_list, int B, int phase, size_t jl_doubles, size_t xyz_doubles, size_t* configured, int num_cus, int tail_below, hipStream_t stream) {
  const size_t head = 512 + (16 * 27 + 5 + 32) * sizeof(double) + 64;
  if (phase == SFTB_PH_INIT) {
    hipError_t e = hipMemsetAsync(d_counters, 0, 16 * sizeof(int), stream);
    if (e != hipSuccess) return e;
    hipLaunchKernelGGL(sftb_init_kernel, dim3(B), dim3(64 * SFTB_NW), 0, stream, d_probs, d_runs, d_counters, d_list, tail_below);
  } else if (phase == SFTB_PH_LIN) {
    const size_t lds = head + jl_doubles * sizeof(double);
    if (lds > configured[0]) {
      hipError_t e = hipFuncSetAttribute(reinterpret_cast<const void*>(sftb_lin_kernel), hipFuncAttributeMaxDynamicSharedMemorySize, (int)lds);
      if (e != hipSuccess) return e;
      configured[0] = lds;
    }
    const int per_cu = lds > 80 * 1024 ? 1 : 2;
    hipLaunchKernelGGL(sftb_lin_kernel, dim3(std::min(B, per_cu * num_cus)), dim3(64 * SFTB_LIN_NW), lds, stream, d_probs, d_runs, d_counters, d_list, B, tail_below);
  } else if (phase == SFTB_PH_FACTOR) {
    hipLaunchKernelGGL(sftb_factor_kernel, dim3(std::min(B, 4 * num_cus)), dim3(64), WV_LDS_DOUBLES * sizeof(double), stream, d_probs, d_runs, d_counters, B);
  } else {
    const size_t lds = head + std::max<size_t>(2048, xyz_doubles) * sizeof(double);
    if (lds > configured[1]) {
      hipError_t e = hipFuncSetAttribute(reinterpret_cast<const void*>(sftb_trial_kernel), hipFuncAttributeMaxDynamicSharedMemorySize, (int)lds);
      if (e != hipSuccess) return e;
      configured[1] = lds;
    }
    hipLaunchKernelGGL(sftb_trial_kernel, dim3(B), dim3(64 * SFTB_NW), lds, stream, d_probs, d_runs, d_counters, d_list);
  }
  return hipGetLastError();
}

#ifdef DSH_LAB
extern "C" hipError_t sftb_factor_lab_launch(const SftDev* d_probs, SftRun* d_runs, int* d_counters, int B, int grid, hipStream_t stream) {
  hipLaunchKernelGGL(sftb_factor_kernel, dim3(grid), dim3(64), WV_LDS_DOUBLES * sizeof(double), stream, d_probs, d_runs, d_counters, B);
  return hipGetLastError();
}
#endif
```

defslam_amd/csrc/sft_plan.h:

```cpp
#pragma once
#include <stddef.h>
#include <stdint.h>

#include <vector>

#include "sft_problem.h"

constexpr int kNB = 32;
constexpr int kTS = 16, kBT = 8, kWB = 16;
constexpr int kSftMaxSub = 4;

struct SftOptions { int waves = 0; int dataflow = 1; int wide_off = 0; int speculate = 0; int split = 2; int rounds = 1; int streams = 0; int helpers = -1; int tail = -1; int owner_waves = 8; int helpers_wbt = 12; };

enum class SftUploadMode { batch, shared_camera, connected };

struct SftSizes { int32_t n, nA, Dn, kd, M, S, Es, max_iters; };

struct SftCut {
  int sT, sp, c0, n1;
  bool room;
};
inline SftCut sft_cut(int Dn, int kd) {
  SftCut c;
  c.sT = (kd + kTS - 1) / kTS;
  c.sp = kTS * c.sT;
  c.c0 = ((Dn - c.sp) / 2 / kTS) * kTS;
  c.n1 = Dn - c.sp - c.c0;
  c.room = c.sT >= 2 && c.c0 >= 4 * kTS && c.n1 >= 4 * kTS;
  return c;
}

struct SftProblemPlan {
  int32_t tile_mode = 0, wbt = 0, tpr = 0;
  bool dataflow = false;
  int32_t lds_class = 0;
  int32_t split = 0, sp_c0 = 0, sp_s = 0, sp_n1p = 0, sp_pad = 0, sp_xl = 0;
  SftPart part[4] = {};
  void apply(SftDev& h) const {
    h.tile_mode = tile_mode; h.wbt = wbt; h.tpr = tpr;
    h.mode = (h.mode & ~2) | (dataflow ? 2 : 0);
    h.lds_class = lds_class;
    h.split = split; h.sp_c0 = sp_c0; h.sp_s = sp_s; h.sp_n1p = sp_n1p; h.sp_pad = sp_pad; h.sp_xl = sp_xl;
    for (int g = 0; g < 4; g++) h.part[g] = part[g];
  }
};

struct SftBatchPlan {
  int nw = 8;
  bool rounds_mode = false;
  int n_sub = 1;
  int K = 1;
  int nh = 0;
  bool any_split = false;
  int max_kd = 0;
  size_t jl_doubles = 0;
  size_t xyz_doubles = 0;
  int max_iters_batch = 0;
  std::vector<SftProblemPlan> prob;
};

SftBatchPlan sft_plan_batch(const SftSizes* sizes, int B, int num_cus, const SftOptions& opt, bool host_only, SftUploadMode mode);

struct SftBatchLayout {
  struct ReadOnly { size_t obs_nodes, obs_bary, obs_uv, obs_w, ob_ptr, ob_m, ob_c, viewed, xyz_init, pose_init; };
  struct Result { size_t xyz, chi2, trace, mp, outl; };
  struct Part { size_t Hb, Lb, Lt, LbT, Lbord, Linv, x, xchg, Pf, PfB, sync; };
  struct Work { size_t bak, camrec, wtv, Anode, Jstar, Jstr, Hc, Hb, Hbord, Hcn, Lb, Lbord, Lc, Linv, Lt, LbT, x, dbg, sx0, sx1, shadow_xyz, shadow_chi2, shadow_hdr; Part part[4]; };
  size_t o_tab = 0;
  std::vector<ReadOnly> ro;
  size_t ro_bytes = 0;
  size_t res_off = 0, res_bytes = 0;
  std::vector<Result> res_offs;
  size_t ws_off = 0;
  size_t o_spec = 0;
  size_t o_runs = 0;
  size_t o_sync = 0, sync_total = 0;
  std::vector<Work> ws;
  size_t size = 0;
};
```

defslam_amd/csrc/sft_problem.h:

```cpp
#pragma once
#include <stdint.h>

#define SFT_NT 512
#define SFT_CAM_STRIDE 16
#define SFT_BORDER 7
#define SFT_H_PAD_TILE_ROWS 9
#define SFT_H_PAD_BORDER 160

#define SFT_KIND_OBS 0u
#define SFT_KIND_REF 1u
#define SFT_KIND_STAR 2u
#define SFT_KIND_STR 3u
#define SFT_REC(kind, s, t, e) (((uint32_t)(kind) << 30) | ((uint32_t)(s) << 26) | ((uint32_t)(t) << 22) | (uint32_t)(e))

#if defined(__HIP_DEVICE_COMPILE__) && defined(SFT_KERNEL_SOURCE)
#define SFT_G __attribute__((address_space(1)))
#else
#define SFT_G
#endif

struct SftResHdr {
  int32_t iters, trials, status, inliers;
  double rep_error;
  double pose[8];
  double pad[5];
};

#define SFT_SC_XCHG 32
#define SFT_SC_LIN 0
#define SFT_SC_FAC 1
#define SFT_SC_SOL 2
#define SFT_SC_CTL 3
#define SFT_CN_LIN 0
#define SFT_CN_FAC 1
#define SFT_CN_SOL 2
#define SFT_CN_CTL 3
struct SftSc {
  double send[SFT_SC_XCHG], recv[SFT_SC_XCHG];
  double lambda, ni, chi_cur, chi_ini, rho, lambda_start;
  double bc[6];
  double pose_bak[8];
  int32_t it, qmax, nbad, accepted, again, done, all_ok, fact_ok, iters, trials, rank, nranks;
};

#define SFT_SPEC_MAXK 4
#define SFT_SPEC_INIT 0
#define SFT_SPEC_LIN 1
#define SFT_SPEC_TRIAL 2
#ifndef SFT_WAVES_PER_EU
#define SFT_WAVES_PER_EU 2
#endif
#define SFT_SPEC_FACTOR 3
#define SFT_SPEC_SOLVE 4
struct SftSpecRes { double chi_new, scale, lambda, ni, pose[8]; int32_t ok, valid; };
struct SftSpec {
  double lambda, ni, chi_cur, chi_ini, lambda_start, rho;
  double pose_bak[8];
  int32_t it, qbase, nbad, accepted, all_ok, iters, trials, done, launches, need_lin, last_lane, pad;
  SftSpecRes res[2];
};

#define SFTB_LIN 0
#define SFTB_TRIAL 1
#define SFTB_DONE 2
#define SFTB_FINISH 3
#define SFTB_PH_INIT 0
#define SFTB_PH_LIN 1
#define SFTB_PH_FACTOR 2
#define SFTB_PH_TRIAL 3
#define SFTB_PH_TAIL 4
struct SftRun {
  double lambda, ni, chi_cur, chi_ini, rho, lambda_start;
  double pose_bak[8];
  int32_t it, qmax, nbad, accepted, all_ok, iters, trials, state, fact_ok, pad[3];
};

struct SftPart {
  int32_t nT, nS, tpr, wbt;
  int32_t b_base, b_sign, b_lo, b_hi;
  SFT_G double* Hb;
  SFT_G double *Lb, *Lt, *LbT, *Lbord, *Linv, *x;
  SFT_G double* xchg;
  SFT_G double *Pf, *PfB;
  SFT_G int32_t* sync;
};

struct SftDev {
  int32_t n, nA, Dn, kd, ldh, M, V, S, Es, noff, max_iters, mode;
  int32_t tile_mode;
  int32_t pad1;
  int32_t lds_class;
  int32_t tpr, wbt;
  int32_t pad0;
  double fx, fy, cx, cy;
  double w_ref, w_curv, w_str, hub_delta, hub_dsqr;
  const SFT_G double* xyz0;
  const SFT_G int32_t* nbr_ptr;
  const SFT_G int32_t* nbr_idx;
  const SFT_G double* nbr_w;
  const SFT_G double* nbr_sumw;
  const SFT_G double* k0;
  const SFT_G int32_t* act;
  const SFT_G int32_t* actnode;
  const SFT_G int32_t* star_node;
  const SFT_G double* star_sL;
  const SFT_G int32_t* str_nodes;
  const SFT_G double* str_L0;
  const SFT_G int32_t* off_ptr;
  const SFT_G int32_t* off_rc;
  const SFT_G int32_t* sh_ptr;
  const SFT_G uint32_t* sh_rec;
  const SFT_G double* sh_cf;
  const SFT_G int32_t* tmask;
  const SFT_G uint32_t* hgatherT;
  const SFT_G uint32_t* hgather;
  const SFT_G int32_t* obs_nodes;
  const SFT_G double* obs_bary;
  const SFT_G double* obs_uv;
  const SFT_G double* obs_w;
  const SFT_G int32_t* ob_ptr;
  const SFT_G int32_t* ob_m;
  const SFT_G double* ob_c;
  const SFT_G uint8_t* viewed;
  const SFT_G double* xyz_init;
  const SFT_G double* pose_init;
  SFT_G double* xyz;
  SFT_G double* xyz_bak;
  SFT_G double* pose;
  SFT_G double* camrec;
  SFT_G double* wtv;
  SFT_G double* Anode;
  SFT_G double* Jstar;
  SFT_G double* Jstr;
  SFT_G double* Hc;
  SFT_G double* Hb;
  SFT_G double* Hbord;
  SFT_G double* Hcorner;
  SFT_G double* Lb;
  SFT_G double* Lbord;
  SFT_G double* Lcorner;
  SFT_G double* Linv;
  SFT_G double* Lt;
  SFT_G double* LbT;
  SFT_G double* x;
  SFT_G double* chi2_obs;
  SFT_G double* trace;
  SFT_G SftResHdr* res;
  SFT_G uint8_t* outlier;
  SFT_G float* mappoint;
  SFT_G double* dbg;
  SFT_G double* spec_xyz[2];
  int32_t split;
  int32_t sp_c0, sp_s, sp_n1p, sp_pad;
  int32_t sp_xl;
  int32_t pad2[2];
  SftPart part[4];
};

#include <hip/hip_runtime.h>
#include <stddef.h>
extern "C" size_t sft_lm_kernel_lds_bytes(int kd, size_t jl_doubles);
extern "C" hipError_t sft_lm_launch(const SftDev* d_probs, int B, int max_kd, size_t jl_doubles, int nw, size_t* configured, hipStream_t stream);
extern "C" hipError_t sftb_launch(const SftDev* d_probs, SftRun* d_runs, int* d_counters, int* d_list, int B, int phase, size_t jl_doubles, size_t xyz_doubles,
                                  size_t* configured, int num_cus, int tail_below, hipStream_t stream);
extern "C" hipError_t sftb_tail_launch(const SftDev* d_probs, SftRun* d_runs, int* d_counters, int B, int max_kd, size_t jl_doubles, size_t* configured, int num_cus,
                                       int tail_below, hipStream_t stream);
extern "C" hipError_t sft_spec_launch(const SftDev* d_probs, SftSpec* d_spec, int B, int K, int phase, int nh, int owner_waves, int max_kd, size_t jl_doubles,
                                      size_t* configured, hipStream_t stream);
extern "C" hipError_t sft_sc_launch(const SftDev* d_probs, SftSc* d_sc, int B, int phase, int max_kd, size_t jl_doubles, size_t* configured, hipStream_t stream);
extern "C" hipError_t sft_sc_local_reduce(SftSc* const* d_ptrs, int G, hipStream_t stream);
extern "C" hipError_t sft_cn_launch(const SftDev* d_probs, SftSc* d_sc, int phase, int max_kd, size_t jl_doubles, size_t* configured, hipStream_t stream);
extern "C" hipError_t sft_vec_sum2(const double* a, const double* b, double* out_a, double* out_b, int n, hipStream_t stream);
#ifdef DSH_LAB
extern "C" hipError_t sft_wave_lab_launch(const SftDev* d_probs, int B, int which, double rel, int max_kd, size_t jl_doubles, hipStream_t stream);
extern "C" hipError_t sft_assembly_launch(const SftDev* d_probs, int B, int max_kd, size_t jl_doubles, int nw, hipStream_t stream);
extern "C" hipError_t sftb_factor_lab_launch(const SftDev* d_probs, SftRun* d_runs, int* d_counters, int B, int grid, hipStream_t stream);
#endif
```

defslam_amd/csrc/sft_wave.h:

```cpp
#pragma once

#if defined(WV_STEP_TRACE) && defined(DSH_LAB)
#define WV_T_DECL long long wv_tr[9] = {0, 0, 0, 0, 0, 0, 0, 0, 0}, wv_tl = clock64()
#define WV_T(e) do { const long long t__ = clock64(); wv_tr[e] += t__ - wv_tl; wv_tl = t__; } while (0)
#define WV_T_ARG , long long (&wv_tr)[9], long long& wv_tl
#define WV_T_PASS , wv_tr, wv_tl
#define WV_T_DUMP(P) do { if ((threadIdx.x & 63) == 0) for (int e__ = 0; e__ < 9; e__++) (P).dbg[40 + e__] = (double)wv_tr[e__]; } while (0)
#else
#define WV_T_DECL do {} while (0)
#define WV_T(e) do {} while (0)
#define WV_T_ARG
#define WV_T_PASS
#define WV_T_DUMP(P) do {} while (0)
#endif

__host__ __device__ constexpr int wv_phys(int r, int d) {
  return d == 0 ? r : (d <= 3 ? 8 * d + r : (d == 4 ? 32 + (r & 3) : 8 * (8 - d) + ((r + 8 - d) & 7)));
}
constexpr int WV_AGPR_TILES = 32;
constexpr int WV_L_WIN = 0;
constexpr int WV_L_BORD = 1024;
constexpr int WV_L_WSCR = 2048;
constexpr int WV_L_CN = 2336;
constexpr int WV_L_XRING = 2400;
// ... 575 lines not shown
  }
}
template <int PH, int T0, int TEND>
__device__ __forceinline__ void wv_lds_pipe(const WvState& S, int q8, lds_double* lds, int lane) {
  wv_task_t<T0> C = wv_task_load<PH, T0>(lds, lane);
  wv_task_t<T0 + 1> Cn = wv_task_load<PH, T0 + 1>(lds, lane);
  wv_task_mfma<T0>(C, S, q8);
  wv_lds_pipe_next<PH, T0 + 1, TEND>(S, q8, lds, lane, Cn, C);
}

template <int PH>
__device__ __forceinline__ v4d wv_step_diag(const WvProb& W, int k, int lane) {
  v4d d = wv_read_agpr<wv_phys(PH, 0)>();
  const int g = lane >> 4, c = lane & 15;
#pragma unroll
  for (int q = 0; q < 4; q++)
    if (g + 4 * q == c && TS * k + c < W.Dn) d[q] += W.lambda;
  return d;
}

template <int PH, bool TAIL>
__device__ __forceinline__ void wv_step_rest(const WvProb& W, WvState& S, const v4d& w, int k, lds_double* lds, int lane, const WvPrev& Q WV_T_ARG) {
  lds_double* ldsw = lds + WV_L_WIN;
  lds_double* ldsb = lds + WV_L_BORD;
  lds_double* wscr = lds + WV_L_WSCR;
  const int nT = W.nT;
  WvBO Bk;
  wv_bo_load(ldsb + 128 * PH, lane, Bk);
  const v4d D4 = wv_lds_load(ldsw + 256 * (wv_phys((PH + 4) & 7, 4) - WV_AGPR_TILES), lane);
  v4d Wt;
  {
    const int g = lane >> 4, c = lane & 15;
#pragma unroll
    for (int q = 0; q < 4; q++) wscr[(g + 4 * q) * 17 + c] = w[q];
#pragma unroll
    for (int q = 0; q < 4; q++) Wt[q] = wscr[c * 17 + g + 4 * q];
  }
  WvTri Wq;
  wv_tri_load(wscr, lane, Wq);
  WV_T(2);
  wv_trsm_b4(S.Yq, Wt, Bk);
  wv_trsm_cols<PH, 1, 2>(S, Wq, k, nT, D4, lane);
  wv_bq_store(wscr, lane, S.Yq);
  wv_trsm_cols<PH, 3, 4>(S, Wq, k, nT, D4, lane);
  wv_bo_load(wscr, lane, S.Yo);
  v4d yba, ybs;
  {
    const lds_double* t = wscr + 2 * wv_bo_lane(lane);
    const lds_double* ta = t + (lane >> 3 & 1);
    const lds_double* tb = t + (lane >> 2 & 1);
#pragma unroll
    for (int q = 0; q < 4; q++) { yba[q] = ta[8 * q]; ybs[q] = tb[8 * q]; }
  }
  asm volatile("" :: "v"(D4[0]), "v"(D4[1]), "v"(D4[2]), "v"(D4[3]));
  wv_trsm_cols<PH, 5, 7>(S, Wq, k, nT, D4, lane);
  if (W.q8 == 1) wv_trsm4_vgpr_q1(S.Y[8], Wq, S.araw);
  else wv_trsm_vgpr(S.Y[8], Wt, S.araw, W.q8);
  wv_mfma_fence();
  WV_T(3);
  SFT_G double* col = W.Lg + ((size_t)k * (BT + 1)) * 256;
  v4d fresh4 = wv_gather_vgpr(W, S.rl.o[4]);
  asm volatile("" : "+v"(S.bnext.n0), "+v"(S.bnext.n1));
  wv_bq_store(ldsb + 128 * PH, lane, S.bnext);
  WV_T(4);
  asm volatile("s_nop 1\n\t"
               "v_mfma_f64_4x4x4_4b_f64 %0, %1, %5, %0 neg:[1,0,0]\n\ts_nop 3\n\t"
               "v_mfma_f64_4x4x4_4b_f64 %0, %2, %6, %0 neg:[1,0,0]\n\ts_nop 3\n\t"
               "v_mfma_f64_4x4x4_4b_f64 %0, %3, %7, %0 neg:[1,0,0]\n\ts_nop 3\n\t"
               "v_mfma_f64_4x4x4_4b_f64 %0, %4, %8, %0 neg:[1,0,0]"
               : "+v"(S.corner)
               : "v"(yba[0]), "v"(yba[1]), "v"(yba[2]), "v"(yba[3]), "v"(ybs[0]), "v"(ybs[1]), "v"(ybs[2]), "v"(ybs[3])
               : "memory");
  wv_update_rows<PH, TAIL, 1, 7>(W, S, k, nT, W.q8, col);
  wv_lds_pipe<PH, 0, 9>(S, W.q8, lds, lane);
  WV_T(5);
  wv_wait_vm();
  WV_T(6);
  {
    WvB2 C10 = wv_task_load<PH, 10>(lds, lane);
    wv_update_rows<PH, TAIL, 8, 8>(W, S, k, nT, W.q8, col);
    wv_task_mfma<10>(C10, S, W.q8);
    wv_task_mfma<11>(fresh4, S, W.q8);
    wv_task_store<PH, 10>(lds, lane, C10);
    wv_mfma_fence();
    wv_task_store<PH, 11>(lds, lane, fresh4);
  }
  asm volatile("" : "+v"(S.corner));
  WV_T(8);
}

struct WvTriList { unsigned o[36][4]; };
template <int R, int D>
__device__ __forceinline__ void wv_prologue_lists(const WvProb& W, int lane, WvTriList& T) {
  if constexpr (R < 8) {
    wv_list(W, R, D, lane, T.o[R * (R + 1) / 2 + D]);
    if constexpr (D < R) wv_prologue_lists<R, D + 1>(W, lane, T);
    else wv_prologue_lists<R + 1, 0>(W, lane, T);
  }
}
template <int R, int D>
__device__ __forceinline__ void wv_prologue_gathers(const WvProb& W, WvTriList& T, v4d (&f4)[8]) {
  if constexpr (R < 8) {
    unsigned (&o)[4] = T.o[R * (R + 1) / 2 + D];
    if constexpr (R == 0 && D == 0) {
#pragma unroll
      for (int t = 0; t < 36; t++) asm volatile("" : "+v"(T.o[t][0]), "+v"(T.o[t][1]), "+v"(T.o[t][2]), "+v"(T.o[t][3]));
    }
    if constexpr (D == 4) f4[R] = wv_gather_vgpr(W, o);
    else wv_gather_agpr<wv_phys(R, D)>(W.Hc, o[0], o[1], o[2], o[3]);
    if constexpr (D < R) wv_prologue_gathers<R, D + 1>(W, T, f4);
    else wv_prologue_gathers<R + 1, 0>(W, T, f4);
  }
}
template <int PH>
__device__ __forceinline__ void wv_prologue_store(lds_double* lds, int lane, v4d& f4, WvB2& bd) {
  if constexpr (PH >= 4) {
    asm volatile("" : "+v"(f4));
    wv_lds_store(lds + WV_L_WIN + 256 * (wv_phys(PH, 4) - WV_AGPR_TILES), lane, f4);
  }
  asm volatile("" : "+v"(bd.n0), "+v"(bd.n1));
  wv_bq_store(lds + WV_L_BORD + 128 * PH, lane, bd);
}

__device__ __forceinline__ int wv_factor(const SftDev& P, double lambda, double lam_corner, lds_double* lds, const WvPrev& Q, double& xcam_out) {
  asm volatile("" ::: "a0", "a255");
  int lane;
  asm volatile("v_mbcnt_lo_u32_b32 %0, -1, 0\n\tv_mbcnt_hi_u32_b32 %0, -1, %0" : "=v"(lane));
  const int g = lane >> 4, c = lane & 15;
  WvProb W;
  W.Dn = uni(P.Dn);
  W.Dnp = ((W.Dn + NB - 1) / NB) * NB;
  W.nT = W.Dnp / TS;
  W.q8 = min(3, max(0, (TS * BT - uni(P.kd)) / 4));
  W.m8[0] = wv_granule_mask(4 - (TS * BT - uni(P.kd)));
  W.m8[1] = wv_granule_mask(12 - (TS * BT - uni(P.kd)));
  W.lambda = lambda;
  W.lam_corner = lam_corner;
  W.bofs = (unsigned)((c & 3) * W.Dnp + 4 * (c >> 2) + g);
  W.Hc = uni(P.Hc); W.hgl = uni(P.hgatherT); W.Hbord = uni(P.Hbord); W.Lg = uni(P.Lb); W.Linv = uni(P.Linv);
  lds_double* wscr = lds + WV_L_WSCR;
  lds_double* Cn = lds + WV_L_CN;
#ifdef DSH_LAB
  const long long wv_t0 = clock64();
#endif
  if (Q.active) wv_bs_begin(Q, lds, lane);
  WvState S;
#pragma unroll
  for (int i = 0; i < 9; i++) S.Y[i] = (v4d){0.0, 0.0, 0.0, 0.0};
  const int cr = 4 * (c >> 3) + g, cc = 4 * ((c >> 2) & 1) + (c & 3);
  S.corner = 0.0;
  if (cr < SFT_BORDER && cc < SFT_BORDER && cc <= cr) S.corner = P.Hcorner[cr * 7 + cc] + ((cr == cc && cr < 6) ? lam_corner : 0.0);
  S.ok = 1;
  {
    WvTriList T;
    v4d f4[8];
    WvB2 bd[8];
    wv_prologue_lists<0, 0>(W, lane, T);
    wv_prologue_gathers<0, 0>(W, T, f4);
#pragma unroll
    for (int r = 0; r < 8; r++) bd[r] = wv_border_fresh(W, r, lane);
    wv_list(W, 8, 8, lane, S.al);
    wv_prologue_store<0>(lds, lane, f4[0], bd[0]); wv_prologue_store<1>(lds, lane, f4[1], bd[1]); wv_prologue_store<2>(lds, lane, f4[2], bd[2]);
    wv_prologue_store<3>(lds, lane, f4[3], bd[3]); wv_prologue_store<4>(lds, lane, f4[4], bd[4]); wv_prologue_store<5>(lds, lane, f4[5], bd[5]);
    wv_prologue_store<6>(lds, lane, f4[6], bd[6]); wv_prologue_store<7>(lds, lane, f4[7], bd[7]);
  }
  wv_wait_vm();
  asm volatile("" : "+v"(S.al[0]), "+v"(S.al[1]), "+v"(S.al[2]), "+v"(S.al[3]));
#ifdef DSH_LAB
  const long long wv_t1 = clock64();
  const long long wv_w1 = wall_clock64();
#endif

  WV_T_DECL;
#pragma unroll 1
  for (int k = 0; k < W.nT; k++) {
    const int ph = k & 7;
    asm volatile("v_lshlrev_b32 %0, 4, %1" : "=v"(S.off_lane) : "v"(lane));
    S.araw = wv_gather_vgpr(W, S.al);
    wv_list(W, k + 9, 8, lane, S.al);
    wv_row_list(W, k + 8, lane, S.rl);
    S.bnext = wv_border_fresh(W, k + 8, lane);
    v4d d;
    switch (ph) {
      case 0: d = wv_step_diag<0>(W, k, lane); break;
      case 1: d = wv_step_diag<1>(W, k, lane); break;
      case 2: d = wv_step_diag<2>(W, k, lane); break;
      case 3: d = wv_step_diag<3>(W, k, lane); break;
      case 4: d = wv_step_diag<4>(W, k, lane); break;
      case 5: d = wv_step_diag<5>(W, k, lane); break;
      case 6: d = wv_step_diag<6>(W, k, lane); break;
      default: d = wv_step_diag<7>(W, k, lane); break;
    }
    WV_T(0);
    if (Q.active) {
      const int J = Q.nT - 1 - k;
      if (J >= 0) wv_bs_step(Q, J, lds, lane);
    }
    WV_T(7);
    v4d w;
    if (!wv_chol_inv(d, w)) {
#ifdef DSH_LAB
      if (S.ok && lane == 0) P.dbg[3] = 1000.0 + k;
#endif
      S.ok = 0;
    }
    WV_T(1);
    {
      const SFT_G double* slot = W.Linv + (size_t)k * 256;
      const v2d_w w01 = (v2d_w){w[0], w[1]}, w23 = (v2d_w){w[2], w[3]};
      unsigned long long keep;
      asm volatile("s_and_saveexec_b64 %0, %5\n\tglobal_store_dwordx4 %1, %2, %4\n\ts_mov_b64 exec, %0\n\t"
                   "s_and_saveexec_b64 %0, %6\n\tglobal_store_dwordx4 %1, %3, %4 offset:1024\n\ts_mov_b64 exec, %0"
                   : "=&s"(keep) : "v"(S.off_lane), "v"(w01), "v"(w23), "s"(slot), "s"(WV_MASK_W0), "s"(WV_MASK_W1) : "memory", "scc");
    }
    switch (ph + ((k + 8 >= W.nT) ? 8 : 0)) {
      case 0: wv_step_rest<0, false>(W, S, w, k, lds, lane, Q WV_T_PASS); break;
      case 1: wv_step_rest<1, false>(W, S, w, k, lds, lane, Q WV_T_PASS); break;
      case 2: wv_step_rest<2, false>(W, S, w, k, lds, lane, Q WV_T_PASS); break;
      case 3: wv_step_rest<3, false>(W, S, w, k, lds, lane, Q WV_T_PASS); break;
      case 4: wv_step_rest<4, false>(W, S, w, k, lds, lane, Q WV_T_PASS); break;
      case 5: wv_step_rest<5, false>(W, S, w, k, lds, lane, Q WV_T_PASS); break;
      case 6: wv_step_rest<6, false>(W, S, w, k, lds, lane, Q WV_T_PASS); break;
      case 7: wv_step_rest<7, false>(W, S, w, k, lds, lane, Q WV_T_PASS); break;
      case 8: wv_step_rest<0, true>(W, S, w, k, lds, lane, Q WV_T_PASS); break;
      case 9: wv_step_rest<1, true>(W, S, w, k, lds, lane, Q WV_T_PASS); break;
      case 10: wv_step_rest<2, true>(W, S, w, k, lds, lane, Q WV_T_PASS); break;
      case 11: wv_step_rest<3, true>(W, S, w, k, lds, lane, Q WV_T_PASS); break;
      case 12: wv_step_rest<4, true>(W, S, w, k, lds, lane, Q WV_T_PASS); break;
      case 13: wv_step_rest<5, true>(W, S, w, k, lds, lane, Q WV_T_PASS); break;
      case 14: wv_step_rest<6, true>(W, S, w, k, lds, lane, Q WV_T_PASS); break;
      default: wv_step_rest<7, true>(W, S, w, k, lds, lane, Q WV_T_PASS); break;
    }
  }
  WV_T_DUMP(P);
  if (Q.active) {
    for (int J = Q.nT - 1 - W.nT; J >= 0; J--) { wv_wait_vm(); wv_bs_step(Q, J, lds, lane); }
  }
#ifdef DSH_LAB
  const long long wv_t2 = clock64();
  const long long wv_w2 = wall_clock64();
#endif
  wv_mfma_fence();
  {
    int l2;
    asm volatile("v_mbcnt_lo_u32_b32 %0, -1, 0\n\tv_mbcnt_hi_u32_b32 %0, -1, %0" : "=v"(l2));
    const int g2 = l2 >> 4, c2 = l2 & 15;
    const int cr2 = 4 * (c2 >> 3) + g2, cc2 = 4 * ((c2 >> 2) & 1) + (c2 & 3);
    if (cr2 < SFT_BORDER && cc2 < SFT_BORDER) Cn[cr2 * 7 + cc2] = S.corner;
  }
  double xcam = 0.0;
  {
    int okc = 1;
    if (lane == 0) {
      double xc[6] = {0, 0, 0, 0, 0, 0};
      bool bad = false;
      for (int kk = 0; kk < 6; kk++) {
        double dd = Cn[kk * 7 + kk];
        for (int j = 0; j < kk; j++) dd -= Cn[kk * 7 + j] * Cn[kk * 7 + j];
        if (!(dd > 0.0)) bad = true;
        const double piv = sqrt(dd);
        Cn[kk * 7 + kk] = piv;
        for (int r = kk + 1; r < 7; r++) {
          double v = Cn[r * 7 + kk];
          for (int j = 0; j < kk; j++) v -= Cn[r * 7 + j] * Cn[kk * 7 + j];
          Cn[r * 7 + kk] = v / piv;
        }
      }
      if (bad) okc = 0;
      for (int kk = 5; kk >= 0; kk--) {
        double v = Cn[6 * 7 + kk];
        for (int r = kk + 1; r < 6; r++) v -= Cn[r * 7 + kk] * xc[r];
        xc[kk] = v / Cn[kk * 7 + kk];
      }
      for (int kk = 0; kk < 6; kk++) Cn[49 + kk] = xc[kk];
    }
    okc = __builtin_amdgcn_readfirstlane(okc);
    if (!okc) S.ok = 0;
    if (c < 6) xcam = Cn[49 + c];
  }
  xcam_out = xcam;
#ifdef DSH_LAB
  if (lane == 0) { P.dbg[5] = (double)(wv_t1 - wv_t0); P.dbg[6] = (double)(wv_t2 - wv_t1); P.dbg[4] = (double)(wv_w2 - wv_w1); }
#endif
  return __builtin_amdgcn_readfirstlane(S.ok);
}

__device__ __forceinline__ WvPrev wv_prev_of(const SftDev& P, int ok, double xcam, int lane_) {
  (void)lane_;
  int lane;
  asm volatile("v_mbcnt_lo_u32_b32 %0, -1, 0\n\tv_mbcnt_hi_u32_b32 %0, -1, %0" : "=v"(lane));
  const int c = lane & 15;
  WvPrev Q;
  const int Dn = uni(P.Dn), Dnp = ((Dn + NB - 1) / NB) * NB;
  Q.Lg = uni(P.Lb); Q.Linv = uni(P.Linv); Q.x = uni(P.x);
  Q.nT = Dnp / TS;
  Q.m8[0] = wv_granule_mask(4 - (TS * BT - uni(P.kd)));
  Q.m8[1] = wv_granule_mask(12 - (TS * BT - uni(P.kd)));
  Q.active = ok;
  Q.xb = (c < 6) ? xcam : ((c == 6) ? -1.0 : 0.0);
  if (ok && lane < 6) P.x[Dnp + lane] = xcam;
  return Q;
}

__device__ __forceinline__ int wv_factor_solve(const SftDev& P, double lambda, double lam_corner, lds_double* lds) {
  WvPrev none;
  none.Lg = nullptr; none.Linv = nullptr; none.x = nullptr; none.nT = 0; none.active = 0; none.m8[0] = none.m8[1] = 0; none.xb = 0.0;
  double xcam;
  const int ok = wv_factor(P, lambda, lam_corner, lds, none, xcam);
  int lane;
  asm volatile("v_mbcnt_lo_u32_b32 %0, -1, 0\n\tv_mbcnt_hi_u32_b32 %0, -1, %0" : "=v"(lane));
  const WvPrev Q = wv_prev_of(P, ok, xcam, lane);
#ifdef DSH_LAB
  const long long t2 = clock64();
#endif
  if (ok) wv_backsub_now(Q, lane);
#ifdef DSH_LAB
  if (lane == 0) P.dbg[7] = (double)(clock64() - t2);
#endif
  return ok;
}
```

Measured before the change: 431,900.

## Carry last back-substitution across FACTOR launches and queue problems through a ring

The FACTOR kernel no longer scans every problem for the TRIAL state. It now takes problems from a ring buffer fed by LIN and TRIAL. Each wave can also defer the back-substitution of its last factorisation into the next FACTOR launch (carry mode), so that work overlaps with the next factorisation instead of stalling at the end of the launch. Mode 2 additionally lets FACTOR take only full wave-sets, and problems are held via an entered/held mechanism that feeds the tail kernel. This adds extra states, atomics and a larger round budget, and problems can lag by one launch.

After: 433,600, median of 6. Within noise of the previous version (+0.4%).

```diff
diff --git a/defslam_amd/csrc/dsh_api.cpp b/defslam_amd/csrc/dsh_api.cpp
--- a/defslam_amd/csrc/dsh_api.cpp
+++ b/defslam_amd/csrc/dsh_api.cpp
@@ -164,14 +164,16 @@
     if (c->opt.tail > 0) tail_below = c->opt.tail * c->num_cus;
     else tail_below = std::min(4 * c->num_cus, std::max(2 * c->num_cus, (int)((long long)3 * B / 4)));
   }
+  const int carry = S == 1 ? c->opt.carry : 0;
   auto launch = [&](int s, int phase) {
     const bool ev = c->phase_events && S == 1;
     if (ev) { hipEvent_t e; if (hipEventCreate(&e) == hipSuccess) { (void)hipEventRecord(e, c->stream); c->phase_events->push_back(e); c->phase_ids.push_back(phase); } }
     hipError_t r;
     {
       LDS_LOCK();
-      if (phase == SFTB_PH_TAIL) r = sftb_tail_launch(c->d_probs + b0[s], c->d_runs + b0[s], c->d_counters + 16 * s, b0[s + 1] - b0[s], c->plan.max_kd, c->plan.jl_doubles, &LDS_MARKS(c).tail, c->num_cus, tail_below, c->sub_stream[s]);
-      else r = sftb_launch(c->d_probs + b0[s], c->d_runs + b0[s], c->d_counters + 16 * s, c->d_linlist + b0[s], b0[s + 1] - b0[s], phase, c->plan.jl_doubles, c->plan.xyz_doubles, LDS_MARKS(c).b,
+      const SftbAux aux{c->d_ring + b0[s], c->d_held + b0[s], c->d_entered + (size_t)s * c->n_entered, c->d_carry + b0[s], c->n_entered, carry};
+      if (phase == SFTB_PH_TAIL) r = sftb_tail_launch(c->d_probs + b0[s], c->d_runs + b0[s], c->d_counters + 16 * s, b0[s + 1] - b0[s], c->plan.max_kd, c->plan.jl_doubles, &LDS_MARKS(c).tail, c->num_cus, c->sub_stream[s]);
+      else r = sftb_launch(c->d_probs + b0[s], c->d_runs + b0[s], c->d_counters + 16 * s, c->d_linlist + b0[s], &aux, b0[s + 1] - b0[s], phase, c->plan.jl_doubles, c->plan.xyz_doubles, LDS_MARKS(c).b,
                            c->num_cus, tail_below, c->sub_stream[s]);
     }
     if (ev) { hipEvent_t e; if (hipEventCreate(&e) == hipSuccess) { (void)hipEventRecord(e, c->stream); c->phase_events->push_back(e); } }
@@ -182,8 +184,8 @@
     for (int s = 1; s < S; s++) HIPCHK(c, hipStreamWaitEvent(c->sub_stream[s], c->sub_event[0], 0));
   }
   for (int s = 0; s < S; s++) HIPCHK(c, launch(s, SFTB_PH_INIT));
-  const int worst = std::max(1, c->plan.max_iters_batch) * 10 + 1;
-  int rounds = 0, group = std::max(1, std::min(worst, c->rounds_hint));
+  const int worst = (std::max(1, c->plan.max_iters_batch) * 10 + 1) * (carry ? 2 : 1) + (carry == 2 ? B / std::max(1, 4 * c->num_cus) + 1 : 0);
+  int rounds = 0, group = std::max(1, std::min(worst, c->rounds_hint + (carry ? 2 : 0)));
   if (tail_below >= B) group = 0;
   HIPCHK(c, c->spec_done.ensure(64 * kSftMaxSub, true));
   int rc = DSH_OK;
@@ -276,7 +278,7 @@
   L.ws.resize((size_t)B * K);
   L.ws_off = a.size;
   L.o_spec = a.take(sizeof(SftSpec) * (size_t)B * K);
-  L.o_runs = a.take(plan.rounds_mode ? sizeof(SftRun) * (size_t)B + 64 * kSftMaxSub + sizeof(int) * (size_t)B : 0);
+  L.o_runs = a.take(plan.rounds_mode ? sizeof(SftRun) * (size_t)B + 64 * kSftMaxSub + sizeof(int) * ((size_t)4 * B + (size_t)kSftMaxSub * (std::max(1, plan.max_iters_batch) * 10 + 2)) : 0);
   if (nh > 0)
     for (int e = 0; e < B * K; e++) {
       const SftProblemPlan& p = plan.prob[e % B];
@@ -453,6 +455,8 @@
   c->d_runs = (SftRun*)(base + L.o_runs);
   c->d_counters = (int*)(base + L.o_runs + sizeof(SftRun) * (size_t)B);
   c->d_linlist = c->d_counters + 16 * kSftMaxSub;
+  c->d_ring = c->d_linlist + B; c->d_held = c->d_ring + B; c->d_carry = c->d_held + B; c->d_entered = c->d_carry + B;
+  c->n_entered = std::max(1, plan.max_iters_batch) * 10 + 2;
   c->d_sync = base + L.o_sync;
   c->plan = std::move(plan);
   c->layout = std::move(L);
@@ -708,6 +712,7 @@
   else if (k == "owner_waves") { if (value != 8 && value != 16) return dsh_fail(c, DSH_ERR_ARG, "dsh_lab_set_option: owner_waves is 8 or 16 (wavefronts of a FACTOR workgroup with helpers)"); c->opt.owner_waves = value; }
   else if (k == "helpers") { if (value < -1 || value > 3) return dsh_fail(c, DSH_ERR_ARG, "dsh_lab_set_option: helpers is -1 (automatic) or 0..3 workgroups per part"); c->opt.helpers = value; }
   else if (k == "tail") { if (value < -1 || value > 8) return dsh_fail(c, DSH_ERR_ARG, "dsh_lab_set_option: tail is -1 (automatic), 0 (rounds to the end) or the number of problems per CU from which downwards the last problems go to the tail kernel"); c->opt.tail = value; }
+  else if (k == "carry") { if (value < 0 || value > 2) return dsh_fail(c, DSH_ERR_ARG, "dsh_lab_set_option: carry is 0 (every FACTOR launch finishes its back substitutions), 1 (a wave carries its last one into the next launch) or 2 (and FACTOR takes full wave-sets only)"); c->opt.carry = value; }
   else if (k == "speculate") { if (value < 0 || value > SFT_SPEC_MAXK) return dsh_fail(c, DSH_ERR_ARG, "dsh_lab_set_option: speculate is 0 (automatic) or 1..4 lanes"); c->opt.speculate = value; }
   else return dsh_fail(c, DSH_ERR_ARG, "dsh_lab_set_option: unknown option " + k);
   return DSH_OK;
diff --git a/defslam_amd/csrc/dsh_sft_ctx.h b/defslam_amd/csrc/dsh_sft_ctx.h
--- a/defslam_amd/csrc/dsh_sft_ctx.h
+++ b/defslam_amd/csrc/dsh_sft_ctx.h
@@ -55,6 +55,11 @@
   SftRun* d_runs = nullptr;
   int* d_counters = nullptr;
   int* d_linlist = nullptr;
+  int* d_ring = nullptr;
+  int* d_held = nullptr;
+  int* d_carry = nullptr;
+  int* d_entered = nullptr;
+  int n_entered = 0;
   int rounds_hint = 24;
   hipStream_t sub_stream[kSftMaxSub] = {nullptr, nullptr, nullptr, nullptr};
   hipEvent_t sub_event[kSftMaxSub] = {nullptr, nullptr, nullptr, nullptr};
diff --git a/defslam_amd/csrc/sft_batch.h b/defslam_amd/csrc/sft_batch.h
--- a/defslam_amd/csrc/sft_batch.h
+++ b/defslam_amd/csrc/sft_batch.h
@@ -18,14 +18,43 @@
   panel = out + 32;
 }
 
-__global__ __launch_bounds__(64 * SFTB_NW, 2) void sftb_init_kernel(const SftDev* __restrict__ probs, SftRun* __restrict__ runs, int* __restrict__ counters, int* __restrict__ lin_list, int tail_below) {
+__device__ __forceinline__ void sftb_ring_push(const SftbAux& A, int* counters, int B, int b) { A.ring[atomicAdd(&counters[11], 1) % B] = b; }
+__device__ __forceinline__ void sftb_arrive(SftRun& R, const SftbAux& A, int* counters, int* lin_list, int B, int tail_below, int b, int st) {
+  const int tau = ++R.tau;
+  const int before = atomicAdd(&A.entered[tau], 1);
+  if (before >= tail_below) {
+    if (before == tail_below) { atomicAdd(&counters[4], tail_below); counters[14] = 1; }
+    R.state = st;
+    if (st == SFTB_LIN) lin_list[atomicAdd(&counters[2], 1)] = b; else sftb_ring_push(A, counters, B, b);
+  } else {
+    R.state = st | SFTB_HELD;
+    A.held[atomicAdd(&counters[13], 1)] = b;
+    atomicSub(&counters[4], 1);
+  }
+}
+#ifndef SFTB_LAG_SETS
+#define SFTB_LAG_SETS 2
+#endif
+#ifndef SFTB_LAG_MAX
+#define SFTB_LAG_MAX 2
+#endif
+__device__ __forceinline__ int sftb_take(const int* counters, int W, int carry_mode) {
+  const int E = counters[11] - counters[10];
+  return (carry_mode == 2 && E >= SFTB_LAG_SETS * W) ? E - E % W : E;
+}
+
+__global__ __launch_bounds__(64 * SFTB_NW, 2) void sftb_init_kernel(const SftDev* __restrict__ probs, SftRun* __restrict__ runs, int* __restrict__ counters, int* __restrict__ lin_list, SftbAux A, int tail_below) {
   const SftDev& P = probs[blockIdx.x];
-  if (blockIdx.x == 0 && threadIdx.x == 0 && (int)gridDim.x <= tail_below) counters[6] = 1;
+  if (blockIdx.x == 0 && threadIdx.x == 0) {
+    if ((int)gridDim.x <= tail_below) counters[6] = 1; else counters[4] = gridDim.x;
+    A.entered[1] = gridDim.x;
+  }
   init_state<64 * SFTB_NW>(P);
   if (threadIdx.x == 0) {
+    A.carry[blockIdx.x] = -1;
     SftRun& R = runs[blockIdx.x];
     R.lambda = -1.0; R.ni = 2.0; R.chi_cur = 0.0; R.chi_ini = 0.0; R.rho = 0.0; R.lambda_start = 0.0;
-    R.it = 0; R.qmax = 0; R.nbad = 0; R.accepted = 0; R.all_ok = 1; R.iters = 0; R.trials = 0; R.fact_ok = 1;
+    R.it = 0; R.qmax = 0; R.nbad = 0; R.accepted = 0; R.all_ok = 1; R.iters = 0; R.trials = 0; R.fact_ok = 1; R.tau = 1;
     R.state = P.max_iters > 0 ? SFTB_LIN : SFTB_FINISH;
     if (P.max_iters > 0) lin_list[atomicAdd(&counters[2], 1)] = blockIdx.x;
   }
@@ -53,63 +82,100 @@
 }
 
 __global__ __launch_bounds__(64 * SFTB_LIN_NW, SFTB_LIN_WAVES) void sftb_lin_kernel(const SftDev* __restrict__ probs, SftRun* __restrict__ runs, int* __restrict__ counters,
-                                                                                  const int* __restrict__ lin_list, int B, int tail_below) {
+                                                                                  const int* __restrict__ lin_list, SftbAux A, int B, int tail_below) {
   constexpr int NW = SFTB_LIN_NW, NT = 64 * NW;
   extern __shared__ __attribute__((aligned(16))) char smem[];
   __shared__ int next_b;
   Ctl* ctl; double *red, *out, *panel;
   sftb_ctl_lds(smem, ctl, red, out, panel);
   const int tid = threadIdx.x;
-  if (counters[6] || B - counters[0] <= tail_below) {
+  if (counters[6] || (tail_below >= 0 && counters[4] == 0)) {
     if (blockIdx.x == 0 && tid == 0) counters[6] = 1;
     return;
   }
   if (blockIdx.x == 0 && tid == 0) counters[7]++;
-  auto fetch = [&]() { const int i = atomicAdd(&counters[3], 1); return i < counters[2] ? lin_list[i] : -1; };
+  auto fetch = [&]() {
+    const int i = atomicAdd(&counters[3], 1), n = counters[2];
+    if (i < n) return lin_list[i];
+    if (!counters[14] || i - n >= counters[13]) return -1;
+    const int h = A.held[i - n];
+    return (runs[h].state & ~SFTB_HELD) == SFTB_TRIAL ? h | (1 << 30) : h;
+  };
   int nxt = -1;
   if (tid == 0) nxt = fetch();
   while (true) {
     if (tid == 0) next_b = nxt;
     __syncthreads();
-    const int b = __builtin_amdgcn_readfirstlane(next_b);
-    if (b < 0) break;
-    if (tid == 0) { nxt = fetch(); atomicAdd(&counters[9], 1); }
-    sftb_lin_problem<NW>(probs[b], runs[b], ctl, red, out, panel);
-  }
-}
-
-__global__ __launch_bounds__(64, 1) void sftb_factor_kernel(const SftDev* __restrict__ probs, SftRun* __restrict__ runs, int* __restrict__ counters, int B) {
+    const int e = __builtin_amdgcn_readfirstlane(next_b);
+    if (e < 0) break;
+    const int b = e & ~(1 << 30);
+    int slot = 0;
+    if (tid == 0) { nxt = fetch(); slot = atomicAdd(&counters[11], 1); }
+    if (e == b) {
+      if (tid == 0) atomicAdd(&counters[9], 1);
+      sftb_lin_problem<NW>(probs[b], runs[b], ctl, red, out, panel);
+    } else if (tid == 0) runs[b].state = SFTB_TRIAL;
+    if (tid == 0) A.ring[slot % B] = b;
+  }
+}
+
+__global__ __launch_bounds__(64, 1) void sftb_factor_kernel(const SftDev* __restrict__ probs, SftRun* __restrict__ runs, int* __restrict__ counters, int B, SftbAux A) {
   extern __shared__ __attribute__((aligned(16))) char smem[];
   lds_double* lds = to_lds(reinterpret_cast<double*>(smem));
   const int lane = threadIdx.x;
   if (counters[6]) return;
   for (int i = lane; i < WV_LDS_DOUBLES; i += 64) lds[i] = 0.0;
-  if (blockIdx.x == 0 && lane == 0) { counters[2] = 0; counters[3] = 0; }
-  WvPrev Q;
-  Q.Lg = nullptr; Q.Linv = nullptr; Q.x = nullptr; Q.nT = 0; Q.active = 0; Q.m8[0] = Q.m8[1] = 0; Q.xb = 0.0;
+  const bool scan = A.ring == nullptr, carry = !scan && A.carry_mode != 0;
+  if (blockIdx.x == 0 && lane == 0) {
+    counters[2] = 0; counters[3] = 0;
+    if (counters[14]) { counters[13] = 0; counters[14] = 0; }
+    if (!scan) counters[12] = sftb_take(counters, gridDim.x, A.carry_mode);
+  }
+  WvPrev Q = wv_prev_none();
+  int qb = -1;
+  if (carry) {
+    wv_slot_put(lds, blockIdx.x, lane);
+    qb = A.carry[blockIdx.x];
+    if (qb >= 0) Q = wv_prev_carried(probs[qb], runs[qb].fact_ok);
+  }
   int n_done = 0;
   while (true) {
     int b = 0;
     if (lane == 0) b = atomicAdd(&counters[1], 1);
     b = __builtin_amdgcn_readfirstlane(b);
-    if (b >= B) break;
-    if (runs[b].state != SFTB_TRIAL) continue;
+    if (scan) {
+      if (b >= B) break;
+      if (runs[b].state != SFTB_TRIAL) continue;
+    } else {
+      if (b >= sftb_take(counters, gridDim.x, A.carry_mode)) break;
+      b = __builtin_amdgcn_readfirstlane(A.ring[(unsigned)(counters[10] + b) % (unsigned)B]);
+    }
+    if (lane == 0 && qb >= 0) runs[qb].state = SFTB_XREADY;
     const SftDev& P = probs[b];
     const double lambda = runs[b].lambda;
     double xcam;
     const int ok = wv_factor(P, lambda, lambda, lds, Q, xcam);
-    if (lane == 0) runs[b].fact_ok = ok;
+    if (lane == 0) { runs[b].fact_ok = ok; runs[b].state = SFTB_XOUT; }
     Q = wv_prev_of(P, ok, xcam, lane);
+    qb = b;
     n_done++;
   }
   int lane_now;
   asm volatile("v_mbcnt_lo_u32_b32 %0, -1, 0\n\tv_mbcnt_hi_u32_b32 %0, -1, %0" : "=v"(lane_now));
-  if (Q.active) wv_backsub_now(Q, lane_now);
+  if (qb >= 0) {
+    const bool keep = carry && n_done && sftb_take(counters, gridDim.x, A.carry_mode) >= SFTB_LAG_SETS * (int)gridDim.x && counters[7] - runs[qb].tau < SFTB_LAG_MAX;
+    if (!keep) {
+      if (Q.active) wv_backsub_now(Q, lane_now);
+      if (lane_now == 0) runs[qb].state = SFTB_XREADY;
+    }
+    if (carry && lane_now == 0) A.carry[wv_slot_get(lds)] = keep ? qb : -1;
+  }
   if (lane_now == 0 && n_done) atomicAdd(&counters[8], n_done);
 }
 
 template <int NW>
-__device__ __forceinline__ int sftb_trial_problem(const SftDev& P, SftRun& R, Ctl* ctl, double* red, double* out, double* panel, int* counters, int* lin_list, int b) {
+__device__ __forceinline__ int sftb_trial_problem(const SftDev& P, SftRun& R, Ctl* ctl, double* red, double* out, double* panel, int* counters, int* lin_list, const SftbAux& A, int B,
+                                                  int tail_below, int b) {
   constexpr int NT = 64 * NW;
   const int tid = threadIdx.x;
   const int Dn = P.Dn;
@@ -166,7 +232,10 @@
     for (int i = tid; i < 3 * P.n; i += NT) P.xyz[i] = staged.xyz_l[i];
   }
   const bool again = (ctl->rho < 0) && (ctl->qmax < 10);
-  if (again) return 0;
+  if (again) {
+    if (tid == 0 && lin_list) sftb_arrive(R, A, counters, lin_list, B, tail_below, b, SFTB_TRIAL);
+    return 0;
+  }
   __syncthreads();
   if (tid == 0) {
     const int qmax = R.qmax;
@@ -188,26 +257,29 @@
     ctl->it = R.iters;
     ctl->accepted = R.trials;
     R.state = term ? SFTB_DONE : SFTB_LIN;
-    if (!term && lin_list) lin_list[atomicAdd(&counters[2], 1)] = b;
+    if (!term && lin_list) sftb_arrive(R, A, counters, lin_list, B, tail_below, b, SFTB_LIN);
   }
   __syncthreads();
   if (ctl->nbad) {
     const int iters = ctl->it, trials = ctl->accepted;
     __syncthreads();
     classify<NT>(P, ctl, panel, iters, trials);
-    if (tid == 0) atomicAdd(&counters[0], 1);
+    if (tid == 0) { atomicAdd(&counters[0], 1); if (lin_list) atomicSub(&counters[4], 1); }
     return 2;
   }
   return 1;
 }
 
-__global__ __launch_bounds__(64 * SFTB_NW, SFTB_TRIAL_WAVES) void sftb_trial_kernel(const SftDev* __restrict__ probs, SftRun* __restrict__ runs, int* __restrict__ counters, int* __restrict__ lin_list) {
+__global__ __launch_bounds__(64 * SFTB_NW, SFTB_TRIAL_WAVES) void sftb_trial_kernel(const SftDev* __restrict__ probs, SftRun* __restrict__ runs, int* __restrict__ counters, int* __restrict__ lin_list,
+                                                                                    SftbAux A, int tail_below) {
   constexpr int NW = SFTB_NW, NT = 64 * NW;
   SftRun& R = runs[blockIdx.x];
   const int st = R.state;
   if (counters[6]) return;
-  if (blockIdx.x == 0 && threadIdx.x == 0) counters[1] = 0;
-  if (st != SFTB_TRIAL && st != SFTB_FINISH) return;
+  if (blockIdx.x == 0 && threadIdx.x == 0) {
+    counters[1] = 0; counters[10] += counters[12]; counters[12] = 0;
+  }
+  if (st != SFTB_XREADY && st != SFTB_FINISH) return;
   extern __shared__ __attribute__((aligned(16))) char smem[];
   const SftDev& P = probs[blockIdx.x];
   Ctl* ctl; double *red, *out, *panel;
@@ -215,10 +287,10 @@
   const int tid = threadIdx.x;
   if (st == SFTB_FINISH) {
     classify<NT>(P, ctl, panel, 0, 0);
-    if (tid == 0) { R.state = SFTB_DONE; atomicAdd(&counters[0], 1); }
+    if (tid == 0) { R.state = SFTB_DONE; atomicAdd(&counters[0], 1); atomicSub(&counters[4], 1); }
     return;
   }
-  (void)sftb_trial_problem<NW>(P, R, ctl, red, out, panel, counters, lin_list, blockIdx.x);
+  (void)sftb_trial_problem<NW>(P, R, ctl, red, out, panel, counters, lin_list, A, (int)gridDim.x, tail_below, blockIdx.x);
 }
 
 __device__ __noinline__ void sftb_solve8(const SftDev& P, unsigned ctl_off, unsigned ws_off, double lambda) {
@@ -229,14 +301,14 @@
   backsub_tiles<8>(P, ctl, ws);
 }
 
-__global__ __launch_bounds__(64 * SFTB_NW, SFT_WAVES_PER_EU) void sftb_tail_kernel(const SftDev* __restrict__ probs, SftRun* __restrict__ runs, int* __restrict__ counters, int B, int tail_below) {
+__global__ __launch_bounds__(64 * SFTB_NW, SFT_WAVES_PER_EU) void sftb_tail_kernel(const SftDev* __restrict__ probs, SftRun* __restrict__ runs, int* __restrict__ counters, int B) {
   constexpr int NW = SFTB_NW, NT = 64 * NW;
   extern __shared__ __attribute__((aligned(16))) char smem[];
   Ctl* ctl; double *red, *out, *panel;
   sftb_ctl_lds(smem, ctl, red, out, panel);
   const int tid = threadIdx.x;
   if (!counters[6]) {
-    if (B - counters[0] > tail_below) return;
+    if (counters[4] != 0) return;
     if (blockIdx.x == 0 && tid == 0) counters[6] = 1;
   }
   while (true) {
@@ -254,6 +326,7 @@
       if (tid == 0) { R.state = SFTB_DONE; atomicAdd(&counters[0], 1); }
       continue;
     }
+    if (st != SFTB_DONE) st &= ~SFTB_HELD;
     while (st == SFTB_LIN || st == SFTB_TRIAL) {
       if (st == SFTB_LIN) {
         sftb_lin_problem<NW>(P, R, ctl, red, out, panel);
@@ -264,7 +337,7 @@
       sftb_solve8(P, (unsigned)(size_t)(__attribute__((address_space(3))) char*)(char*)ctl, (unsigned)(size_t)(__attribute__((address_space(3))) char*)(char*)panel, R.lambda);
       if (tid == 0) R.fact_ok = ctl->fact_ok;
       __syncthreads();
-      const int r = sftb_trial_problem<NW>(P, R, ctl, red, out, panel, counters, nullptr, b);
+      const int r = sftb_trial_problem<NW>(P, R, ctl, red, out, panel, counters, nullptr, SftbAux{}, B, -1, b);
       __syncthreads();
       st = r == 0 ? SFTB_TRIAL : (r == 1 ? SFTB_LIN : SFTB_DONE);
     }
diff --git a/defslam_amd/csrc/sft_kernels.hip b/defslam_amd/csrc/sft_kernels.hip
--- a/defslam_amd/csrc/sft_kernels.hip
+++ b/defslam_amd/csrc/sft_kernels.hip
@@ -2975,14 +2975,14 @@
   return hipGetLastError();
 }
 
-extern "C" hipError_t sftb_tail_launch(const SftDev* d_probs, SftRun* d_runs, int* d_counters, int B, int max_kd, size_t jl_doubles, size_t* configured, int num_cus, int tail_below, hipStream_t stream) {
+extern "C" hipError_t sftb_tail_launch(const SftDev* d_probs, SftRun* d_runs, int* d_counters, int B, int max_kd, size_t jl_doubles, size_t* configured, int num_cus, hipStream_t stream) {
   const size_t lds = sft_lm_kernel_lds_bytes(max_kd, jl_doubles);
   if (lds > *configured) {
     hipError_t e = hipFuncSetAttribute(reinterpret_cast<const void*>(sftb_tail_kernel), hipFuncAttributeMaxDynamicSharedMemorySize, (int)lds);
     if (e != hipSuccess) return e;
     *configured = lds;
   }
-  hipLaunchKernelGGL(sftb_tail_kernel, dim3(std::min(B, num_cus)), dim3(64 * SFTB_NW), lds, stream, d_probs, d_runs, d_counters, B, tail_below);
+  hipLaunchKernelGGL(sftb_tail_kernel, dim3(std::min(B, num_cus)), dim3(64 * SFTB_NW), lds, stream, d_probs, d_runs, d_counters, B);
   return hipGetLastError();
 }
 
@@ -3099,12 +3099,14 @@
 }
 #endif
 
-extern "C" hipError_t sftb_launch(const SftDev* d_probs, SftRun* d_runs, int* d_counters, int* d_list, int B, int phase, size_t jl_doubles, size_t xyz_doubles, size_t* configured, int num_cus, int tail_below, hipStream_t stream) {
+extern "C" hipError_t sftb_launch(const SftDev* d_probs, SftRun* d_runs, int* d_counters, int* d_list, const SftbAux* aux, int B, int phase, size_t jl_doubles, size_t xyz_doubles, size_t* configured, int num_cus, int tail_below, hipStream_t stream) {
   const size_t head = 512 + (16 * 27 + 5 + 32) * sizeof(double) + 64;
   if (phase == SFTB_PH_INIT) {
     hipError_t e = hipMemsetAsync(d_counters, 0, 16 * sizeof(int), stream);
     if (e != hipSuccess) return e;
-    hipLaunchKernelGGL(sftb_init_kernel, dim3(B), dim3(64 * SFTB_NW), 0, stream, d_probs, d_runs, d_counters, d_list, tail_below);
+    e = hipMemsetAsync(aux->entered, 0, (size_t)aux->n_entered * sizeof(int), stream);
+    if (e != hipSuccess) return e;
+    hipLaunchKernelGGL(sftb_init_kernel, dim3(B), dim3(64 * SFTB_NW), 0, stream, d_probs, d_runs, d_counters, d_list, *aux, tail_below);
   } else if (phase == SFTB_PH_LIN) {
     const size_t lds = head + jl_doubles * sizeof(double);
     if (lds > configured[0]) {
@@ -3113,9 +3115,9 @@
       configured[0] = lds;
     }
     const int per_cu = lds > 80 * 1024 ? 1 : 2;
-    hipLaunchKernelGGL(sftb_lin_kernel, dim3(std::min(B, per_cu * num_cus)), dim3(64 * SFTB_LIN_NW), lds, stream, d_probs, d_runs, d_counters, d_list, B, tail_below);
+    hipLaunchKernelGGL(sftb_lin_kernel, dim3(std::min(B, per_cu * num_cus)), dim3(64 * SFTB_LIN_NW), lds, stream, d_probs, d_runs, d_counters, d_list, *aux, B, tail_below);
   } else if (phase == SFTB_PH_FACTOR) {
-    hipLaunchKernelGGL(sftb_factor_kernel, dim3(std::min(B, 4 * num_cus)), dim3(64), WV_LDS_DOUBLES * sizeof(double), stream, d_probs, d_runs, d_counters, B);
+    hipLaunchKernelGGL(sftb_factor_kernel, dim3(std::min(B, 4 * num_cus)), dim3(64), WV_LDS_DOUBLES * sizeof(double), stream, d_probs, d_runs, d_counters, B, *aux);
   } else {
     const size_t lds = head + std::max<size_t>(2048, xyz_doubles) * sizeof(double);
     if (lds > configured[1]) {
@@ -3123,14 +3125,14 @@
       if (e != hipSuccess) return e;
       configured[1] = lds;
     }
-    hipLaunchKernelGGL(sftb_trial_kernel, dim3(B), dim3(64 * SFTB_NW), lds, stream, d_probs, d_runs, d_counters, d_list);
+    hipLaunchKernelGGL(sftb_trial_kernel, dim3(B), dim3(64 * SFTB_NW), lds, stream, d_probs, d_runs, d_counters, d_list, *aux, tail_below);
   }
   return hipGetLastError();
 }
 
 #ifdef DSH_LAB
 extern "C" hipError_t sftb_factor_lab_launch(const SftDev* d_probs, SftRun* d_runs, int* d_counters, int B, int grid, hipStream_t stream) {
-  hipLaunchKernelGGL(sftb_factor_kernel, dim3(grid), dim3(64), WV_LDS_DOUBLES * sizeof(double), stream, d_probs, d_runs, d_counters, B);
+  hipLaunchKernelGGL(sftb_factor_kernel, dim3(grid), dim3(64), WV_LDS_DOUBLES * sizeof(double), stream, d_probs, d_runs, d_counters, B, SftbAux{});
   return hipGetLastError();
 }
 #endif
diff --git a/defslam_amd/csrc/sft_plan.h b/defslam_amd/csrc/sft_plan.h
--- a/defslam_amd/csrc/sft_plan.h
+++ b/defslam_amd/csrc/sft_plan.h
@@ -10,7 +10,7 @@
 constexpr int kTS = 16, kBT = 8, kWB = 16;
 constexpr int kSftMaxSub = 4;
 
-struct SftOptions { int waves = 0; int dataflow = 1; int wide_off = 0; int speculate = 0; int split = 2; int rounds = 1; int streams = 0; int helpers = -1; int tail = -1; int owner_waves = 8; int helpers_wbt = 12; };
+struct SftOptions { int waves = 0; int dataflow = 1; int wide_off = 0; int speculate = 0; int split = 2; int rounds = 1; int streams = 0; int helpers = -1; int tail = -1; int owner_waves = 8; int helpers_wbt = 12; int carry = 2; };
 
 enum class SftUploadMode { batch, shared_camera, connected };
 
diff --git a/defslam_amd/csrc/sft_problem.h b/defslam_amd/csrc/sft_problem.h
--- a/defslam_amd/csrc/sft_problem.h
+++ b/defslam_amd/csrc/sft_problem.h
@@ -64,6 +64,9 @@
 #define SFTB_TRIAL 1
 #define SFTB_DONE 2
 #define SFTB_FINISH 3
+#define SFTB_XOUT 4
+#define SFTB_XREADY 5
+#define SFTB_HELD 8
 #define SFTB_PH_INIT 0
 #define SFTB_PH_LIN 1
 #define SFTB_PH_FACTOR 2
@@ -72,7 +75,15 @@
 struct SftRun {
   double lambda, ni, chi_cur, chi_ini, rho, lambda_start;
   double pose_bak[8];
-  int32_t it, qmax, nbad, accepted, all_ok, iters, trials, state, fact_ok, pad[3];
+  int32_t it, qmax, nbad, accepted, all_ok, iters, trials, state, fact_ok, tau, pad[2];
+};
+struct SftbAux {
+  int* ring;
+  int* held;
+  int* entered;
+  int* carry;
+  int n_entered;
+  int carry_mode;
 };
 
 struct SftPart {
@@ -161,10 +172,10 @@
 #include <stddef.h>
 extern "C" size_t sft_lm_kernel_lds_bytes(int kd, size_t jl_doubles);
 extern "C" hipError_t sft_lm_launch(const SftDev* d_probs, int B, int max_kd, size_t jl_doubles, int nw, size_t* configured, hipStream_t stream);
-extern "C" hipError_t sftb_launch(const SftDev* d_probs, SftRun* d_runs, int* d_counters, int* d_list, int B, int phase, size_t jl_doubles, size_t xyz_doubles,
-                                  size_t* configured, int num_cus, int tail_below, hipStream_t stream);
+extern "C" hipError_t sftb_launch(const SftDev* d_probs, SftRun* d_runs, int* d_counters, int* d_list, const SftbAux* aux, int B, int phase, size_t jl_doubles,
+                                  size_t xyz_doubles, size_t* configured, int num_cus, int tail_below, hipStream_t stream);
 extern "C" hipError_t sftb_tail_launch(const SftDev* d_probs, SftRun* d_runs, int* d_counters, int B, int max_kd, size_t jl_doubles, size_t* configured, int num_cus,
-                                       int tail_below, hipStream_t stream);
+                                       hipStream_t stream);
 extern "C" hipError_t sft_spec_launch(const SftDev* d_probs, SftSpec* d_spec, int B, int K, int phase, int nh, int owner_waves, int max_kd, size_t jl_doubles,
                                       size_t* configured, hipStream_t stream);
 extern "C" hipError_t sft_sc_launch(const SftDev* d_probs, SftSc* d_sc, int B, int phase, int max_kd, size_t jl_doubles, size_t* configured, hipStream_t stream);
diff --git a/defslam_amd/csrc/sft_wave.h b/defslam_amd/csrc/sft_wave.h
--- a/defslam_amd/csrc/sft_wave.h
+++ b/defslam_amd/csrc/sft_wave.h
@@ -901,6 +901,34 @@
   return Q;
 }
 
+__device__ __forceinline__ WvPrev wv_prev_none() {
+  WvPrev Q;
+  Q.Lg = nullptr; Q.Linv = nullptr; Q.x = nullptr; Q.nT = 0; Q.active = 0; Q.m8[0] = Q.m8[1] = 0; Q.xb = 0.0;
+  return Q;
+}
+__device__ __forceinline__ WvPrev wv_prev_carried(const SftDev& P, int ok) {
+  int lane;
+  asm volatile("v_mbcnt_lo_u32_b32 %0, -1, 0\n\tv_mbcnt_hi_u32_b32 %0, -1, %0" : "=v"(lane));
+  const int c = lane & 15;
+  WvPrev Q;
+  const int Dn = uni(P.Dn), Dnp = ((Dn + NB - 1) / NB) * NB;
+  Q.Lg = uni(P.Lb); Q.Linv = uni(P.Linv); Q.x = uni(P.x);
+  Q.nT = Dnp / TS;
+  Q.m8[0] = wv_granule_mask(4 - (TS * BT - uni(P.kd)));
+  Q.m8[1] = wv_granule_mask(12 - (TS * BT - uni(P.kd)));
+  Q.active = __builtin_amdgcn_readfirstlane(ok);
+  Q.xb = (c < 6) ? P.x[Dnp + c] : ((c == 6) ? -1.0 : 0.0);
+  return Q;
+}
+constexpr int WV_L_SLOT = WV_L_CN + 56;
+static_assert(WV_L_SLOT < WV_L_XRING, "the slot word lies between the corner and the x ring");
+__device__ __forceinline__ void wv_slot_put(lds_double* lds, int slot, int lane) {
+  if (lane == 0) *reinterpret_cast<__attribute__((address_space(3))) int*>(lds + WV_L_SLOT) = slot;
+}
+__device__ __forceinline__ int wv_slot_get(const lds_double* lds) {
+  return __builtin_amdgcn_readfirstlane(*reinterpret_cast<const __attribute__((address_space(3))) int*>(lds + WV_L_SLOT));
+}
+
 __device__ __forceinline__ int wv_factor_solve(const SftDev& P, double lambda, double lam_corner, lds_double* lds) {
   WvPrev none;
   none.Lg = nullptr; none.Linv = nullptr; none.x = nullptr; none.nT = 0; none.active = 0; none.m8[0] = none.m8[1] = 0; none.xb = 0.0;
```
